# prajwaljpj/GUAVA_renderer

Measured on AMD Instinct MI355X. Metric: rendered frames/sec @512x512, ~100k Gaussians, higher is better.
Workload: dtype f32; 1 GPU; guava-avatar-synth-100k-512-deform+raster; pipeline=EHM LBS -> Gaussian assembly -> rasterize, gaussians=100000, channels=32, global_batch=32, parallelism=frame-sharded x1, batches_in_flight=4, placement=shared, exp=exact-poly, colour_accum=f32 mfma (bit-exact)

## Files before the change

guava_renderer_amd/_lib.py:

```python
import ctypes
import os

HERE = os.path.dirname(os.path.abspath(__file__))
LIB_PATH = os.path.join(HERE, "lib", "libgsr.so")

EXPORTS = ("gsr_version", "gsr_last_error", "gsr_geometry_bytes",
           "gsr_image_bytes", "gsr_binning_bytes", "gsr_mark_visible", "gsr_forward", "gsr_forward_ex",
           "gsr_forward_async_bound", "gsr_forward_async",
           "gsr_backward", "gsr_backward_ex", "gsr_batch_workspace_bytes", "gsr_forward_batch",
           "gsr_backward_batch", "gsr_backward_batch_shared", "gsr_batch_status", "gsr_profile_enable", "gsr_profile_read",
           "gsr_render_counters", "gsr_render_timeline", "gsr_forward_batch_refine", "gsr_render_variant",
           "gsr_refine_prepare", "gsr_batch_status_offset", "gsr_frames_to8b",
           "gsr_refine_backward_scratch_bytes", "gsr_refine_backward_image", "gsr_refine_backward_rows",
           "gsr_stream_create_cu_mask", "gsr_stream_destroy", "gsr_set_render_stream",
           "gsr_lbs_workspace_bytes", "gsr_lbs", "gsr_lbs_sp", "gsr_blend_joints", "gsr_blend_joints_sp",
           "gsr_lbs_tiled_floats", "gsr_lbs_tile_bases",
           "gsr_scratch_geometry", "gsr_scratch_binning", "gsr_scratch_image", "gsr_forward_batch_deformed",
           "gsr_forward_batch_deformed_refine",
           "gsr_splice_head",
           "gsr_pack_rows", "gsr_deform_gaussians", "gsr_ehm_workspace_bytes", "gsr_ehm_forward",
           "gsr_deform_gaussians_backward", "gsr_backward_batch_deformed",
           "gsr_fused_ssim", "gsr_fused_ssim_backward", "gsr_image_loss_partials", "gsr_image_loss",
           "gsr_guava_loss_workspace_bytes", "gsr_guava_loss_partials", "gsr_guava_loss_forward",
           "gsr_guava_loss_backward", "gsr_uv_regularizers_partials", "gsr_uv_regularizers",
           "gsr_mesh_raster_workspace_bytes", "gsr_mesh_raster", "gsr_mesh_visible_texels",
           "gsr_mesh_raster_stats",
           "gsr_lift_vertices", "gsr_lift_uv", "gsr_lift_backward_workspace_bytes",
           "gsr_lift_vertices_backward", "gsr_lift_uv_backward")

NUMERICS_EXACT = 0
NUMERICS_FAST_EXP = 1
NUMERICS_SPLIT_BF16 = 2
FORWARD_ONLY = 0x100
RENDER_VARIANTS = ("strip", "strip_fwd", "split_frame", "split_shared", "split_shared_fwd", "refine", "refine_fwd",
                   "quad", "quad_refine", "half", "half_split", "stats", "timeline", "quad_timeline")


def numerics(fast_exp=False, split_bf16=False):
    return (NUMERICS_FAST_EXP if fast_exp else 0) | (NUMERICS_SPLIT_BF16 if split_bf16 else 0)


ALLOC_FN = ctypes.CFUNCTYPE(ctypes.c_void_p, ctypes.c_void_p, ctypes.c_size_t)

_vp = ctypes.c_void_p
_i = ctypes.c_int
_i64 = ctypes.c_int64
_f = ctypes.c_float
_sz = ctypes.c_size_t
_u32 = ctypes.c_uint32

_lib = None


class RefineEpilogue(ctypes.Structure):
    _fields_ = [("weight", _vp), ("bias", _vp), ("n_out", _i), ("negative_slope", _f),
                ("out_refine", _vp), ("keep_channels", _i)]


class RefineBackwardDesc(ctypes.Structure):
    _fields_ = [("weight", _vp), ("n_out", _i), ("keep_channels", _i), ("negative_slope", _f), ("pad_", _i),
                ("out_refine", _vp), ("dL_dout_refine", _vp), ("dL_dkeep", _vp), ("dL_dprepared", _vp),
                ("scratch", _vp)]


class Scratch(ctypes.Structure):
    _fields_ = [("geometry", _vp), ("geometry_cap", _sz), ("binning", _vp), ("binning_cap", _sz),
                ("image", _vp), ("image_cap", _sz)]


class DeformInputs(ctypes.Structure):
    _fields_ = [("V", _i), ("F", _i), ("N", _i), ("pad_", _i), ("verts", _vp), ("vert_transforms", _vp),
                ("faces", _vp), ("vtx_rotations", _vp), ("vtx_rot_stride", _i64), ("vtx_scales", _vp),
                ("vtx_scale_stride", _i64), ("binding_face", _vp), ("face_bary", _vp), ("local_xyz", _vp),
                ("local_stride", _i64), ("uv_rotations", _vp), ("uv_rot_stride", _i64), ("uv_scales", _vp),
                ("uv_scale_stride", _i64), ("bad_index_flag", _vp)]


class DeformGrads(ctypes.Structure):
    _fields_ = [("vtx_rotations", _vp), ("vtx_scales", _vp), ("local_xyz", _vp), ("uv_rotations", _vp),
                ("uv_scales", _vp)]


class RowSegment(ctypes.Structure):
    _fields_ = [("src", _vp), ("dst", _vp), ("src_stride", _i64), ("dst_stride", _i64), ("width", _i),
                ("pad_", _i)]


class LbsSparse(ctypes.Structure):
    _fields_ = [("jreg_row", _vp), ("jreg_col", _vp), ("jreg_val", _vp), ("skin_k", ctypes.c_int32),
                ("pad_", ctypes.c_int32), ("skin_joint", _vp), ("skin_weight", _vp),
                ("shapedirs_tiled", _vp), ("posedirs_tiled", _vp), ("shapedirs_tiled_k", ctypes.c_int32),
                ("shapedirs_tiled_m", ctypes.c_int32), ("posedirs_tiled_k", ctypes.c_int32),
                ("posedirs_tiled_m", ctypes.c_int32)]


class EhmModel(ctypes.Structure):
    _fields_ = [("V", ctypes.c_int32), ("J", ctypes.c_int32), ("NB", ctypes.c_int32), ("pad_", ctypes.c_int32),
                ("v_template", _vp), ("shapedirs_t", _vp), ("posedirs", _vp), ("J_regressor", _vp),
                ("lbs_weights_t", _vp), ("parents_host", _vp), ("sparse", ctypes.POINTER(LbsSparse))]


class Ehm(ctypes.Structure):
    _fields_ = [("flame", EhmModel), ("body", EhmModel), ("head_index", _vp), ("l_eyelid", _vp),
                ("r_eyelid", _vp), ("N_head", ctypes.c_int32), ("hj0", ctypes.c_int32), ("hj1", ctypes.c_int32),
                ("bj0", ctypes.c_int32), ("bj1", ctypes.c_int32), ("pad_", ctypes.c_int32), ("bad_index_flag", _vp)]


class EhmParam(ctypes.Structure):
    _fields_ = [("p", _vp), ("row_stride", _i64), ("width", ctypes.c_int32), ("pad_", ctypes.c_int32)]


class EhmOutputs(ctypes.Structure):
    _fields_ = [("vertices", _vp), ("joints", _vp), ("joints_transform", _vp), ("ver_transform_mat", _vp),
                ("joint_transform_mat", _vp)]


EHM_SLOTS = ("flame.shape_params", "flame.expression_params", "flame.jaw_params", "flame.eye_pose_params",
             "flame.eyelid_params", "body.shape", "body.exp", "body.global_pose", "body.body_pose",
             "body.left_hand_pose", "body.right_hand_pose", "body.head_scale", "body.joints_offset")


class GsrError(RuntimeError):
    pass


class CapacityError(GsrError):
    """A batched forward needed more Gaussian-tile instances than its workspace holds (that call's
    images were filled with NaN)."""


def load(path=None):
    global _lib
    if _lib is not None:
        return _lib
    path = path or os.environ.get("GSR_LIB") or LIB_PATH
    import torch
    if not os.path.exists(path):
        try:
            from . import build as _build
            _build.build(verbose=False)
        except Exception as e:
            raise GsrError(f"libgsr.so not found at {path} and could not be built: {e}") from e
    L = ctypes.CDLL(path)
    L.gsr_version.restype = ctypes.c_char_p
    built = L.gsr_version().decode().split()[-1]
    if path == LIB_PATH and os.environ.get("GSR_ALLOW_STALE") != "1":
        from . import build as _build
        if os.path.isdir(_build.CSRC) and built != _build.source_hash():
            raise GsrError(f"{path} was built from other sources (hash {built}, tree {_build.source_hash()}): "
                           "rebuild with `python -m guava_renderer_amd.build` (GSR_ALLOW_STALE=1 overrides)")
    L.gsr_last_error.restype = ctypes.c_char_p
    L.gsr_geometry_bytes.argtypes = [_i, _i, _i]
    L.gsr_geometry_bytes.restype = _sz
    L.gsr_image_bytes.argtypes = [_i, _i]
    L.gsr_image_bytes.restype = _sz
    L.gsr_binning_bytes.argtypes = [_i64]
    L.gsr_binning_bytes.restype = _sz
    L.gsr_mark_visible.argtypes = [_i, _vp, _vp, _vp, _vp, _vp]
    L.gsr_mark_visible.restype = _i
    L.gsr_forward.argtypes = [ALLOC_FN, ALLOC_FN, ALLOC_FN, _vp, _i, _i, _i, _vp, _i, _i, _vp, _vp,
                              _vp, _vp, _vp, _f, _vp, _vp, _vp, _vp, _vp, _f, _f, _i, _vp, _vp, _i,
                              _vp, _i, _vp]
    L.gsr_forward.restype = _i
    L.gsr_forward_ex.argtypes = list(L.gsr_forward.argtypes[:-1]) + [_u32, _vp]
    L.gsr_forward_ex.restype = _i
    L.gsr_forward_async_bound.argtypes = [_i, _i, _i]
    L.gsr_forward_async_bound.restype = _i64
    L.gsr_forward_async.argtypes = list(L.gsr_forward.argtypes[:-1]) + [_vp, _u32, _vp]
    L.gsr_forward_async.restype = _i
    L.gsr_backward.argtypes = [_i, _i, _i, _i, _vp, _i, _i, _vp, _vp, _vp, _vp, _vp, _f, _vp, _vp,
                               _vp, _vp, _vp, _f, _f, _vp, _vp, _vp, _vp, _vp, _vp, _vp, _vp, _vp,
                               _vp, _vp, _vp, _vp, _vp, _vp, _vp, _i, _i, _vp]
    L.gsr_backward.restype = _i
    L.gsr_backward_ex.argtypes = list(L.gsr_backward.argtypes[:-1]) + [_u32, _vp]
    L.gsr_backward_ex.restype = _i
    L.gsr_batch_workspace_bytes.argtypes = [_i, _i, _i, _i, _i64]
    L.gsr_batch_workspace_bytes.restype = _sz
    L.gsr_batch_status_offset.argtypes = [_i, _i, _i, _i, _i64]
    L.gsr_batch_status_offset.restype = _sz
    L.gsr_forward_batch.argtypes = [_i, _i, _i, _i, _vp, _i64, _vp, _i64, _vp, _i64, _vp, _i64, _vp,
                                    _i64, _f, _vp, _vp, _vp, _vp, _i64, _vp, _i64, _vp, _vp, _vp, _i,
                                    _u32, _vp]
    L.gsr_forward_batch.restype = _i
    L.gsr_forward_batch_refine.argtypes = list(L.gsr_forward_batch.argtypes[:-2]) + [
        ctypes.POINTER(RefineEpilogue), _u32, _vp]
    L.gsr_forward_batch_refine.restype = _i
    L.gsr_forward_batch_deformed.argtypes = [_i, _i, _i, ctypes.POINTER(DeformInputs), _vp, _i64, _vp, _i64, _f,
                                             _vp, _vp, _vp, _vp, _i64, _vp, _i64, _vp, _vp, _vp, _i, _u32, _vp]
    L.gsr_forward_batch_deformed.restype = _i
    L.gsr_forward_batch_deformed_refine.argtypes = list(L.gsr_forward_batch_deformed.argtypes[:-2]) + [
        ctypes.POINTER(RefineEpilogue), _u32, _vp]
    L.gsr_forward_batch_deformed_refine.restype = _i
    L.gsr_render_variant.argtypes = [_i, _u32, _i]
    L.gsr_render_variant.restype = _i
    L.gsr_refine_prepare.argtypes = [_i, _vp, _vp, _i, _i, _vp, _vp]
    L.gsr_refine_prepare.restype = _i
    L.gsr_refine_backward_scratch_bytes.argtypes = [_i, _i, _i, _i, _i]
    L.gsr_refine_backward_scratch_bytes.restype = _sz
    L.gsr_refine_backward_image.argtypes = [_i, _i, _i, _i, _vp, _i64, ctypes.POINTER(RefineBackwardDesc), _vp]
    L.gsr_refine_backward_image.restype = _i
    L.gsr_refine_backward_rows.argtypes = [_i, _i, _vp, _vp, _i64, _i, _vp, _vp, _i64,
                                           ctypes.POINTER(RefineBackwardDesc), _vp, _vp, _vp, _vp]
    L.gsr_refine_backward_rows.restype = _i
    L.gsr_backward_batch.argtypes = [_i, _i, _i, _i, _vp, _i64, _vp, _i64, _vp, _i64, _vp, _i64, _vp,
                                     _i64, _f, _vp, _vp, _vp, _vp, _i64, _vp, _i64, _vp, _vp, _vp, _vp,
                                     _vp, _vp, _vp, _vp, _vp, _vp, _vp, _i, _u32, _vp]
    L.gsr_backward_batch.restype = _i
    L.gsr_backward_batch_shared.argtypes = list(L.gsr_backward_batch.argtypes[:24]) + [_vp, _vp, _vp, _vp, _vp,
                                                                                       _i, _u32, _vp]
    L.gsr_backward_batch_shared.restype = _i
    L.gsr_batch_status.argtypes = [_vp, _i, _i, ctypes.POINTER(_i64), ctypes.POINTER(_i), _vp]
    L.gsr_batch_status.restype = _i
    L.gsr_profile_enable.argtypes = [ctypes.c_uint32]
    L.gsr_profile_enable.restype = _i
    L.gsr_profile_read.argtypes = [ctypes.POINTER(ctypes.c_double), ctypes.POINTER(_i), _i]
    L.gsr_profile_read.restype = _i
    L.gsr_render_counters.argtypes = [_vp]
    L.gsr_render_counters.restype = _i
    L.gsr_render_timeline.argtypes = [_vp, ctypes.c_uint32]
    L.gsr_render_timeline.restype = _i
    L.gsr_frames_to8b.argtypes = [_i, _i, _i, _i, _vp, _i64, _vp, _vp]
    L.gsr_frames_to8b.restype = _i
    L.gsr_stream_create_cu_mask.argtypes = [_u32, ctypes.POINTER(_u32), ctypes.POINTER(_vp)]
    L.gsr_stream_create_cu_mask.restype = _i
    L.gsr_stream_destroy.argtypes = [_vp]
    L.gsr_stream_destroy.restype = _i
    L.gsr_set_render_stream.argtypes = [_vp, _vp]
    L.gsr_set_render_stream.restype = _i
    L.gsr_lbs_workspace_bytes.argtypes = [_i, _i, _i, _i]
    L.gsr_lbs_workspace_bytes.restype = _sz
    L.gsr_lbs_tiled_floats.argtypes = [_i, _i]
    L.gsr_lbs_tiled_floats.restype = _sz
    L.gsr_lbs_tile_bases.argtypes = [_i, _i, _vp, _vp, _vp]
    L.gsr_lbs_tile_bases.restype = _i
    L.gsr_lbs.argtypes = [_i, _i, _i, _i, _vp, _i64, _vp, _vp, _vp, _i, _vp, _vp, _vp, _vp, _vp, _vp,
                          _vp, _vp, _vp, _vp, _vp, _vp, _vp]
    L.gsr_lbs.restype = _i
    L.gsr_lbs_sp.argtypes = [_i, _i, _i, _i, _vp, _i64, _vp, _vp, _vp, _i, _vp, _vp, _vp, _vp, _vp, _vp,
                             _vp, _vp, _vp, _vp, _vp, _vp, ctypes.POINTER(LbsSparse), _vp]
    L.gsr_lbs_sp.restype = _i
    L.gsr_blend_joints.argtypes = [_i, _i, _i, _i, _vp, _i64, _vp, _vp, _vp, _vp, _vp, _vp, _vp]
    L.gsr_blend_joints.restype = _i
    L.gsr_blend_joints_sp.argtypes = [_i, _i, _i, _i, _vp, _i64, _vp, _vp, _vp, _vp, _vp, _vp,
                                      ctypes.POINTER(LbsSparse), _vp]
    L.gsr_blend_joints_sp.restype = _i
    L.gsr_splice_head.argtypes = [_i, _i, _i, _vp, _vp, _vp, _vp, _vp, _vp, _vp, _i, _i, _i, _vp, _i,
                                  _i, _i, _vp, _vp, _vp]
    L.gsr_splice_head.restype = _i
    L.gsr_pack_rows.argtypes = [_i, _i, ctypes.POINTER(RowSegment), _vp]
    L.gsr_pack_rows.restype = _i
    L.gsr_deform_gaussians.argtypes = [_i, _i, _i, _i, _vp, _vp, _vp, _vp, _i64, _vp, _i64, _vp, _vp,
                                       _vp, _i64, _vp, _i64, _vp, _i64, _vp, _vp, _vp, _vp, _vp]
    L.gsr_deform_gaussians.restype = _i
    L.gsr_deform_gaussians_backward.argtypes = [_i, ctypes.POINTER(DeformInputs), _vp, _vp, _vp,
                                                ctypes.POINTER(DeformGrads), _vp]
    L.gsr_deform_gaussians_backward.restype = _i
    L.gsr_backward_batch_deformed.argtypes = [_i, _i, _i, ctypes.POINTER(DeformInputs), _vp, _vp, _vp, _vp, _i64,
                                              _vp, _i64, _f, _vp, _vp, _vp, _vp, _i64, _vp, _i64, _vp, _vp, _vp,
                                              _vp, ctypes.POINTER(DeformGrads), _i, _u32, _vp]
    L.gsr_backward_batch_deformed.restype = _i
    L.gsr_ehm_workspace_bytes.argtypes = [ctypes.POINTER(Ehm), _i]
    L.gsr_ehm_workspace_bytes.restype = _sz
    L.gsr_ehm_forward.argtypes = [ctypes.POINTER(Ehm), _i, ctypes.POINTER(EhmParam), ctypes.POINTER(EhmOutputs),
                                  _vp, _vp]
    L.gsr_ehm_forward.restype = _i
    L.gsr_fused_ssim.argtypes = [_i, _i, _i, _i, _f, _f, _vp, _vp, _vp, _vp, _vp, _vp, _vp]
    L.gsr_fused_ssim.restype = _i
    L.gsr_fused_ssim_backward.argtypes = [_i, _i, _i, _i, _f, _f, _vp, _vp, _vp, _vp, _vp, _vp, _vp, _vp]
    L.gsr_fused_ssim_backward.restype = _i
    L.gsr_image_loss_partials.argtypes = [_i, _i, _i]
    L.gsr_image_loss_partials.restype = _i
    L.gsr_image_loss.argtypes = [_i, _i, _i, _vp, _vp, _vp, _f, _f, _vp, _vp, _vp, _vp]
    L.gsr_image_loss.restype = _i
    L.gsr_guava_loss_workspace_bytes.argtypes = [_i, _i, _i, _i, _i]
    L.gsr_guava_loss_workspace_bytes.restype = _sz
    L.gsr_guava_loss_partials.argtypes = [_i, _i, _i, _i, _i]
    L.gsr_guava_loss_partials.restype = _i
    L.gsr_guava_loss_forward.argtypes = [_i, _i, _i, _vp, _vp, _vp, _f, _f, _vp, _f, _i, _i, _i, _vp, _vp, _vp,
                                         _vp, _vp, _vp, _vp, _vp]
    L.gsr_guava_loss_forward.restype = _i
    L.gsr_guava_loss_backward.argtypes = [_i, _i, _i, _vp, _f, _f, _vp, _i, _i, _i, _vp, _vp, _vp, _vp, _vp, _vp]
    L.gsr_guava_loss_backward.restype = _i
    L.gsr_uv_regularizers_partials.argtypes = [_i]
    L.gsr_uv_regularizers_partials.restype = _i
    L.gsr_uv_regularizers.argtypes = [_i, _vp, _vp, _f, _f, _f, _f, _vp, _vp, _vp, _vp]
    L.gsr_uv_regularizers.restype = _i
    L.gsr_mesh_raster_workspace_bytes.argtypes = [_i, _i, _i, _i, _i]
    L.gsr_mesh_raster_workspace_bytes.restype = _sz
    L.gsr_mesh_raster.argtypes = [_i, _i, _i, _i, _i, _vp, _vp, _vp, _vp, _vp, _i, _vp, _vp, _vp, _vp, _vp, _vp]
    L.gsr_mesh_raster.restype = _i
    L.gsr_mesh_visible_texels.argtypes = [_i, _i, _i, _vp, _vp, _vp, _vp]
    L.gsr_mesh_visible_texels.restype = _i
    L.gsr_mesh_raster_stats.argtypes = [_vp, ctypes.POINTER(_i64)]
    L.gsr_mesh_raster_stats.restype = _i
    L.gsr_lift_vertices.argtypes = [_i] * 5 + [_vp] * 8
    L.gsr_lift_vertices.restype = _i
    L.gsr_lift_uv.argtypes = [_i] * 7 + [_vp] * 11
    L.gsr_lift_uv.restype = _i
    L.gsr_lift_backward_workspace_bytes.argtypes = [_i, _i, _i, _i]
    L.gsr_lift_backward_workspace_bytes.restype = _sz
    L.gsr_lift_vertices_backward.argtypes = [_i] * 5 + [_vp] * 8
    L.gsr_lift_vertices_backward.restype = _i
    L.gsr_lift_uv_backward.argtypes = [_i] * 7 + [_vp] * 12
    L.gsr_lift_uv_backward.restype = _i
    _lib = L
    return L


def render_variant(B, numerics=0, refine=False):
    return RENDER_VARIANTS[check(load().gsr_render_variant(int(B), int(numerics), int(bool(refine))),
                                 "gsr_render_variant")]


def check(rc, what):
    if rc < 0:
        msg = load().gsr_last_error().decode(errors="replace")
        raise GsrError(f"{what} failed ({-rc}): {msg}")
    return rc
```

guava_renderer_amd/batch.py:

```python
import ctypes
import weakref

import torch

from . import _lib

C = 32
STAGES = ("preprocess", "scan", "depth_sort", "chunk_count", "tile_scan", "ordered_scatter", "render_fwd",
          "render_bwd", "preprocess_bwd")


def _frame_arg(t, B, P, per, name, device, align16=False):
    if not isinstance(t, torch.Tensor):
        raise TypeError(f"{name} must be a tensor")
    if t.device != device:
        raise ValueError(f"{name} must be on {device} (got {t.device})")
    if t.dtype != torch.float32:
        raise TypeError(f"{name} must be float32 (got {t.dtype})")
    if t.dim() == 2:
        if tuple(t.shape) != (P, per):
            raise ValueError(f"{name}: expected [{P},{per}] or [{B},{P},{per}], got {list(t.shape)}")
        t = t.contiguous()
        return t, 0
    if t.dim() != 3 or tuple(t.shape) != (B, P, per):
        raise ValueError(f"{name}: expected [{P},{per}] or [{B},{P},{per}], got {list(t.shape)}")
    if t.stride(0) == 0:
        row = t[0]
        if not row.is_contiguous():
            row = row.contiguous()
        return row, 0
    dense_rows = t.stride(2) == 1 and (t.stride(1) == per or P == 1)
    fs = t.stride(0)
    if not dense_rows or fs < P * per or (align16 and (fs % 4 or t.data_ptr() % 16)):
        t = t.contiguous()
        fs = P * per
    return t, fs


def _frame_mat(t, B, n, name, device):
    if t.device != device or t.dtype != torch.float32:
        raise ValueError(f"{name} must be float32 on {device}")
    if t.numel() != B * n:
        raise ValueError(f"{name}: expected {B}x{n} floats, got shape {list(t.shape)}")
    return t.contiguous()


class BatchRasterizer:

    def __init__(self, B, P, W, H, R_capacity=None, device="cuda", numerics=0):
        self.B, self.P, self.W, self.H = int(B), int(P), int(W), int(H)
        self.device = torch.device(device)
        if self.device.type == "cuda" and self.device.index is None:
            self.device = torch.device("cuda", torch.cuda.current_device())
        self.R_capacity = int(R_capacity if R_capacity is not None else 16 * P * B)
        self.numerics = int(numerics)
        self.L = _lib.load()
        nbytes = self.L.gsr_batch_workspace_bytes(self.B, self.P, self.W, self.H, self.R_capacity)
        soff = self.L.gsr_batch_status_offset(self.B, self.P, self.W, self.H, self.R_capacity)
        self.workspace = torch.empty((nbytes,), dtype=torch.uint8, device=self.device)
        self._sticky = self.workspace[soff:soff + 16].view(torch.int32)
        self._sticky.zero_()
        self._overflow = self.workspace[4:8].view(torch.int32).reshape(())
        self._status_host = torch.zeros(4, dtype=torch.int32, pin_memory=True)
        self._status_ev = None
        self._fwd_count = 0
        self.out_color = torch.empty((self.B, C, self.H, self.W), dtype=torch.float32, device=self.device)
        self.out_invdepth = torch.empty((self.B, self.H, self.W), dtype=torch.float32, device=self.device)
        self.radii = torch.empty((self.B, self.P), dtype=torch.int32, device=self.device)

    def _stream(self):
        return ctypes.c_void_p(torch.cuda.current_stream(self.device).cuda_stream)

    def _inputs(self, means3D, colors, opacities, scales, rotations, viewmatrices, projmatrices,
                tanfov, backgrounds):
        B, P, dev = self.B, self.P, self.device
        none = (None, 0)
        m, sm = none if means3D is None else _frame_arg(means3D, B, P, 3, "means3D", dev)
        c, sc = _frame_arg(colors, B, P, C, "colors", dev, align16=True)
        o, so = _frame_arg(opacities, B, P, 1, "opacities", dev)
        s, ss = none if scales is None else _frame_arg(scales, B, P, 3, "scales", dev)
        r, sr = none if rotations is None else _frame_arg(rotations, B, P, 4, "rotations", dev)
        v = _frame_mat(viewmatrices, B, 16, "viewmatrices", dev)
        pm = _frame_mat(projmatrices, B, 16, "projmatrices", dev)
        tf = _frame_mat(tanfov, B, 2, "tanfov", dev)
        if backgrounds.device != dev or backgrounds.dtype != torch.float32:
            raise ValueError(f"backgrounds must be float32 on {dev}")
        if backgrounds.dim() == 2:
            if tuple(backgrounds.shape) != (B, C):
                raise ValueError(f"backgrounds: expected [{C}] or [{B},{C}], got {list(backgrounds.shape)}")
            bg = backgrounds.contiguous() if backgrounds.stride(0) != 0 else backgrounds[0].contiguous()
            bs = C if backgrounds.stride(0) != 0 else 0
        elif tuple(backgrounds.shape) == (C,):
            bg, bs = backgrounds.contiguous(), 0
        else:
            raise ValueError(f"backgrounds: expected [{C}] or [{B},{C}], got {list(backgrounds.shape)}")
        keep = (m, c, o, s, r, v, pm, tf, bg)
        ptr = lambda t: None if t is None else t.data_ptr()
        args = (B, P, self.W, self.H, ptr(m), sm, c.data_ptr(), sc, o.data_ptr(), so, ptr(s), ss, ptr(r), sr)
        return keep, args, (v.data_ptr(), pm.data_ptr(), tf.data_ptr(), bg.data_ptr(), bs)

    def _after_forward(self):
        self._fwd_count += 1
        self._status_host.copy_(self._sticky, non_blocking=True)
        ev = torch.cuda.Event()
        ev.record(torch.cuda.current_stream(self.device))
        self._status_ev = ev

    def poll(self, wait=False):
        ev = self._status_ev
        if ev is None:
            return
        if wait:
            ev.synchronize()
        elif not ev.query():
            return
        if int(self._status_host[0]):
            rmax = int(self._status_host[1]) & 0xFFFFFFFF
            self.overflow_need = max(getattr(self, "overflow_need", 0), rmax)
            self._sticky.zero_()
            self._status_host.zero_()
            raise _lib.CapacityError(
                f"batch needed {rmax} Gaussian-tile instances, workspace holds {self.R_capacity} "
                f"(that forward's images are NaN); allocate a BatchRasterizer with a larger R_capacity")

    def max_instances_seen(self):
        return max(int(self._status_host[1]) & 0xFFFFFFFF, getattr(self, "overflow_need", 0))

    def overflow_flag(self):
        return self._overflow

    def forward(self, means3D, colors, opacities, scales, rotations, viewmatrices, projmatrices,
                tanfov, backgrounds, scale_modifier=1.0, antialiasing=False, refine=None, numerics=None,
                forward_only=False):
        self.poll()
        nm = self.numerics if numerics is None else int(numerics)
        if forward_only:
            nm |= _lib.FORWARD_ONLY
        self._fwd_only = bool(forward_only)
        keep, head, (v, pm, tf, bg, bs) = self._inputs(means3D, colors, opacities, scales, rotations,
                                                       viewmatrices, projmatrices, tanfov, backgrounds)
        args = head + (float(scale_modifier), v, pm, tf, bg, bs, self.workspace.data_ptr(), self.R_capacity,
                       self.out_color.data_ptr(), self.out_invdepth.data_ptr(), self.radii.data_ptr(),
                       int(bool(antialiasing)))
        if refine is None:
            _lib.check(self.L.gsr_forward_batch(*args, nm, self._stream()), "gsr_forward_batch")
        else:
            pc = refine.prepare(keep[1], self._stream())
            bgrows = keep[8].reshape(-1, C)
            pb = refine.prepare(bgrows, self._stream(), cache=False)
            args = list(args)
            args[6] = pc.data_ptr()
            args[18] = pb.data_ptr()
            ep = refine.epilogue(self.B, self.H, self.W)
            _lib.check(self.L.gsr_forward_batch_refine(*args, ctypes.byref(ep), nm, self._stream()),
                       "gsr_forward_batch_refine")
        del keep
        self._after_forward()
        return self.out_color, self.out_invdepth, self.radii

    def forward_deformed(self, deformer, verts, vert_transforms, viewmatrices, projmatrices, tanfov, backgrounds,
                         scale_modifier=1.0, antialiasing=False, numerics=None, refine=None):
        self.poll()
        nm = self.numerics if numerics is None else int(numerics)
        self._fwd_only = True
        dfm = deformer
        B, P = self.B, self.P
        if dfm.V + dfm.N != P:
            raise ValueError(f"deformer has {dfm.V + dfm.N} Gaussians, the rasterizer {P}")
        if tuple(verts.shape) != (B, dfm.V, 3) or tuple(vert_transforms.shape) != (B, dfm.V, 4, 4):
            raise ValueError("verts / vert_transforms: expected [B,V,3] / [B,V,4,4]")
        for name, t_ in (("verts", verts), ("vert_transforms", vert_transforms), ("deformer.faces", dfm.faces),
                         ("deformer.colors", dfm.colors), ("deformer.bind", dfm.bind)):
            if t_.device != self.device:
                raise ValueError(f"{name} is on {t_.device}, the rasterizer on {self.device}")
        vb = verts.detach().to(torch.float32).contiguous()
        vt = vert_transforms.detach().to(torch.float32).contiguous()
        keep, head, (v, pm, tf, bg, bs) = self._inputs(None, dfm.colors, dfm.opacity, None, None, viewmatrices,
                                                       projmatrices, tanfov, backgrounds)
        di = _lib.DeformInputs(dfm.V, dfm.faces.shape[0], dfm.N, 0, vb.data_ptr(), vt.data_ptr(),
                               dfm.faces.data_ptr(), dfm.v_rot.data_ptr(), 0, dfm.v_scale.data_ptr(), 0,
                               dfm.bind.data_ptr(), dfm.bary.data_ptr(), dfm.u_local.data_ptr(), 0,
                               dfm.u_rot.data_ptr(), 0, dfm.u_scale.data_ptr(), 0, dfm.bad.data_ptr())
        args = (B, self.W, self.H, ctypes.byref(di), head[6], head[7], head[8], head[9], float(scale_modifier),
                v, pm, tf, bg, bs, self.workspace.data_ptr(), self.R_capacity, self.out_color.data_ptr(),
                self.out_invdepth.data_ptr(), self.radii.data_ptr(), int(bool(antialiasing)))
        if refine is None:
            _lib.check(self.L.gsr_forward_batch_deformed(*args, nm, self._stream()), "gsr_forward_batch_deformed")
        else:
            pc = refine.prepare(keep[1], self._stream())
            pb = refine.prepare(keep[8].reshape(-1, C), self._stream(), cache=False)
            args = list(args)
            args[4] = pc.data_ptr()
            args[12] = pb.data_ptr()
            ep = refine.epilogue(B, self.H, self.W)
            _lib.check(self.L.gsr_forward_batch_deformed_refine(*args, ctypes.byref(ep), nm, self._stream()),
                       "gsr_forward_batch_deformed_refine")
        del keep, vb, vt
        self._after_forward()
        return self.out_color, self.out_invdepth, self.radii

    def backward(self, means3D, colors, opacities, scales, rotations, viewmatrices, projmatrices,
                 tanfov, backgrounds, dL_dcolor, dL_dinvdepth=None, scale_modifier=1.0,
                 antialiasing=False, shared=False, numerics=None):
        B, P = self.B, self.P
        if getattr(self, "_fwd_only", False):
            raise _lib.GsrError("backward after forward(forward_only=True): the workspace holds no backward rows")
        nm = self.numerics if numerics is None else int(numerics)
        o = dict(dtype=torch.float32, device=self.device)
        keep, head, (v, pm, tf, bg, bs) = self._inputs(means3D, colors, opacities, scales, rotations,
                                                       viewmatrices, projmatrices, tanfov, backgrounds)
        if tuple(dL_dcolor.shape) != (B, C, self.H, self.W):
            raise ValueError(f"dL_dcolor: expected [{B},{C},{self.H},{self.W}], got {list(dL_dcolor.shape)}")
        dLc = dL_dcolor.to(torch.float32).contiguous()
        dLi = None
        if dL_dinvdepth is not None:
            if dL_dinvdepth.numel() != B * self.H * self.W:
                raise ValueError("dL_dinvdepth: expected [B,H,W]")
            dLi = dL_dinvdepth.to(torch.float32).contiguous()
        if shared:
            strides = head[5::2]
            if any(st_ != 0 for st_ in strides):
                raise ValueError("backward(shared=True) needs attributes shared by every frame "
                                 "([P,k] tensors or frame stride 0); got per-frame inputs")
            g = dict(colors=torch.zeros((P, C), **o), opacity=torch.empty((P, 1), **o),
                     means3D=torch.empty((P, 3), **o), scales=torch.empty((P, 3), **o),
                     rotations=torch.empty((P, 4), **o))
            rc = self.L.gsr_backward_batch_shared(
                *head, float(scale_modifier), v, pm, tf, bg, bs, self.workspace.data_ptr(), self.R_capacity,
                dLc.data_ptr(), dLi.data_ptr() if dLi is not None else None, g["opacity"].data_ptr(),
                g["colors"].data_ptr(), g["means3D"].data_ptr(), g["scales"].data_ptr(),
                g["rotations"].data_ptr(), int(bool(antialiasing)), nm, self._stream())
            _lib.check(rc, "gsr_backward_batch_shared")
            del keep
            return g
        g = dict(mean2D=torch.zeros((B, P, 3), **o), conic=torch.zeros((B, P, 4), **o),
                 opacity=torch.zeros((B, P, 1), **o), colors=torch.zeros((B, P, C), **o),
                 invdepth=torch.zeros((B, P, 1), **o) if dL_dinvdepth is not None else None,
                 means3D=torch.zeros((B, P, 3), **o), cov3D=torch.zeros((B, P, 6), **o),
                 scales=torch.zeros((B, P, 3), **o), rotations=torch.zeros((B, P, 4), **o))
        rc = self.L.gsr_backward_batch(
            *head, float(scale_modifier), v, pm, tf, bg, bs, self.workspace.data_ptr(), self.R_capacity,
            dLc.data_ptr(), dLi.data_ptr() if dLi is not None else None,
            g["mean2D"].data_ptr(), g["conic"].data_ptr(), g["opacity"].data_ptr(),
            g["colors"].data_ptr(), g["invdepth"].data_ptr() if g["invdepth"] is not None else None,
            g["means3D"].data_ptr(), g["cov3D"].data_ptr(), g["scales"].data_ptr(),
            g["rotations"].data_ptr(), int(bool(antialiasing)), nm, self._stream())
        _lib.check(rc, "gsr_backward_batch")
        del keep
        return g

    def _bg_arg(self, backgrounds):
        if backgrounds.device != self.device or backgrounds.dtype != torch.float32:
            raise ValueError(f"backgrounds must be float32 on {self.device}")
        if tuple(backgrounds.shape) == (C,):
            return backgrounds.contiguous().reshape(1, C), 0
        if backgrounds.dim() != 2 or tuple(backgrounds.shape) != (self.B, C):
            raise ValueError(f"backgrounds: expected [{C}] or [{self.B},{C}], got {list(backgrounds.shape)}")
        if backgrounds.stride(0) == 0:
            return backgrounds[0].contiguous().reshape(1, C), 0
        return backgrounds.contiguous(), C

    def refine_backward_image(self, head, dL_drefined, dL_draw=None, out_refine=None):
        B, P, H, W = self.B, self.P, self.H, self.W
        if getattr(self, "_fwd_only", False):
            raise _lib.GsrError("backward after a forward-only forward: the workspace holds no backward rows")
        out = head.out if out_refine is None else out_refine
        if out is None or tuple(out.shape) != (B, head.n_out, H, W):
            raise ValueError(f"out_refine: expected the refine forward's [{B},{head.n_out},{H},{W}] output")
        if tuple(dL_drefined.shape) != (B, head.n_out, H, W):
            raise ValueError(f"dL_drefined: expected [{B},{head.n_out},{H},{W}], got {list(dL_drefined.shape)}")
        if out.device != self.device or dL_drefined.device != self.device:
            raise ValueError(f"out_refine / dL_drefined must be on {self.device}")
        out = out.to(torch.float32).contiguous()
        dout = dL_drefined.to(torch.float32).contiguous()
        dkeep = None
        if dL_draw is not None and head.keep_channels > 0:
            if tuple(dL_draw.shape) != (B, head.keep_channels, H, W) or dL_draw.device != self.device:
                raise ValueError(f"dL_draw: expected [{B},{head.keep_channels},{H},{W}] on {self.device}")
            dkeep = dL_draw.to(torch.float32).contiguous()
        nbytes = max(self.L.gsr_refine_backward_scratch_bytes(B, W, H, P, 1),
                     self.L.gsr_refine_backward_scratch_bytes(B, W, H, B * P, B))
        scratch = torch.empty((nbytes,), dtype=torch.uint8, device=self.device)
        G = torch.empty((B, C, H, W), dtype=torch.float32, device=self.device)
        desc = _lib.RefineBackwardDesc(head.weight.data_ptr(), head.n_out, head.keep_channels, head.slope, 0,
                                       out.data_ptr(), dout.data_ptr(),
                                       dkeep.data_ptr() if dkeep is not None else None, G.data_ptr(),
                                       scratch.data_ptr())
        _lib.check(self.L.gsr_refine_backward_image(B, P, W, H, self.workspace.data_ptr(), self.R_capacity,
                                                    ctypes.byref(desc), self._stream()),
                   "gsr_refine_backward_image")
        del out, dout, dkeep
        return G, scratch

    def refine_backward_rows(self, head, d_prepared, raw_rows, backgrounds, scratch):
        B, P, dev = self.B, self.P, self.device
        raw, rs = _frame_arg(raw_rows, B, P, C, "raw_rows", dev, align16=True)
        if d_prepared.dtype != torch.float32 or d_prepared.device != dev or \
                tuple(d_prepared.shape) not in ((P, C), (B, P, C)):
            raise ValueError(f"d_prepared: expected float32 [{P},{C}] or [{B},{P},{C}] on {dev}")
        frames = 1 if d_prepared.dim() == 2 else B
        if frames == 1 and rs != 0:
            raise ValueError("frame-reduced d_prepared [P,32] needs raw rows shared by every frame")
        dp = d_prepared.contiguous()
        bg, bs = self._bg_arg(backgrounds)
        need = self.L.gsr_refine_backward_scratch_bytes(B, self.W, self.H, dp.numel() // C, frames)
        if scratch.numel() < need:
            raise ValueError("scratch is not the one refine_backward_image returned for this rasterizer")
        o = dict(dtype=torch.float32, device=dev)
        rows = torch.empty_like(dp)
        dW = torch.empty((head.n_out, C), **o)
        db = torch.empty((head.n_out,), **o)
        desc = _lib.RefineBackwardDesc(head.weight.data_ptr(), head.n_out, head.keep_channels, head.slope, 0,
                                       None, None, None, None, scratch.data_ptr())
        _lib.check(self.L.gsr_refine_backward_rows(dp.numel() // C, frames, dp.data_ptr(), raw.data_ptr(), rs, B,
                                                   scratch.data_ptr(), bg.data_ptr(), bs, ctypes.byref(desc),
                                                   rows.data_ptr(), dW.data_ptr(), db.data_ptr(), self._stream()),
                   "gsr_refine_backward_rows")
        del raw, bg, dp
        return rows, dW, db

    def _prepared(self, head, colors, backgrounds):
        raw, _ = _frame_arg(colors, self.B, self.P, C, "colors", self.device, align16=True)
        bg, bs = self._bg_arg(backgrounds)
        pc = head.prepare(raw, self._stream())
        pb = head.prepare(bg, self._stream(), cache=False)
        return pc, (pb if bs else pb[0])

    def backward_refine(self, head, means3D, colors, opacities, scales, rotations, viewmatrices, projmatrices,
                        tanfov, backgrounds, dL_drefined, dL_draw=None, dL_dinvdepth=None, scale_modifier=1.0,
                        antialiasing=False, shared=False, numerics=None, out_refine=None):
        G, scratch = self.refine_backward_image(head, dL_drefined, dL_draw, out_refine)
        pc, pb = self._prepared(head, colors, backgrounds)
        g = self.backward(means3D, pc, opacities, scales, rotations, viewmatrices, projmatrices, tanfov, pb, G,
                          dL_dinvdepth, scale_modifier=scale_modifier, antialiasing=antialiasing, shared=shared,
                          numerics=numerics)
        g["colors"], g["weight"], g["bias"] = self.refine_backward_rows(head, g["colors"], colors, backgrounds,
                                                                        scratch)
        return g

    def backward_deformed(self, deformer, verts, vert_transforms, deformed, colors, opacities, viewmatrices,
                          projmatrices, tanfov, backgrounds, dL_dcolor=None, dL_dinvdepth=None, scale_modifier=1.0,
                          antialiasing=False, numerics=None, refine=None, dL_drefined=None, dL_draw=None):
        if refine is not None:
            if dL_drefined is None or dL_dcolor is not None:
                raise ValueError("backward_deformed(refine=head) takes dL_drefined (and dL_draw), not dL_dcolor")
            G, scratch = self.refine_backward_image(refine, dL_drefined, dL_draw)
            pc, pb = self._prepared(refine, colors, backgrounds)
            g = self.backward_deformed(deformer, verts, vert_transforms, deformed, pc, opacities, viewmatrices,
                                       projmatrices, tanfov, pb, G, dL_dinvdepth, scale_modifier=scale_modifier,
# ... 194 lines not shown
```

guava_renderer_amd/csrc/capi.hip:

```cpp
#include <cstdio>
#include <cstdlib>
#include <cstring>
#include <mutex>
#include <string>
#include <unordered_map>
#include <vector>

#include "../../include/gsr.h"
#include "../../include/gsr_deform.h"

#include "gsr_internal.h"

using namespace gsr;

namespace {

thread_local std::string g_err;
uint64_t* g_render_counters = nullptr;
uint32_t* g_timeline = nullptr;
uint32_t g_timeline_cap = 0;

int fail(gsr_status st, const std::string& msg) {
    g_err = msg;
    return -(int)st;
// ... 16 lines not shown

constexpr int kStages = GSR_NUM_STAGES;
uint32_t g_prof_mask = 0;
struct EvPair { hipEvent_t a, b; int stage; };
std::vector<EvPair> g_ev_pool;
size_t g_ev_used = 0;
double g_prof_ms[kStages] = {0};
int g_prof_cnt[kStages] = {0};

struct StageTimer {
    EvPair* p = nullptr;
    hipStream_t s;
    StageTimer(int stage, hipStream_t st) : s(st) {
        if (!(g_prof_mask & (1u << stage))) return;
        if (g_ev_used == g_ev_pool.size()) {
            EvPair e;
            if (hipEventCreate(&e.a) != hipSuccess || hipEventCreate(&e.b) != hipSuccess) return;
            g_ev_pool.push_back(e);
        }
        p = &g_ev_pool[g_ev_used++];
        p->stage = stage;
        hipEventRecord(p->a, s);
    }
    ~StageTimer() {
        if (p) hipEventRecord(p->b, s);
    }
};

inline bool exact_exp(uint32_t numerics) { return (numerics & GSR_NUMERICS_FAST_EXP) == 0; }
inline bool split_bf16(uint32_t numerics) { return (numerics & GSR_NUMERICS_SPLIT_BF16) != 0; }
constexpr uint32_t kNumericsKnown = GSR_NUMERICS_FAST_EXP | GSR_NUMERICS_SPLIT_BF16;
constexpr uint32_t kForwardBatchKnown = kNumericsKnown | GSR_FORWARD_ONLY;

inline size_t align_up(size_t x) { return (x + 255) & ~(size_t)255; }
inline size_t ctrl_words(const Dims& d) { return (size_t)kCtrlWords + (size_t)kFsWords * d.B; }

std::string grid_error(int width, int height) {
    if ((int64_t)((width + 15) / 16) * ((height + 15) / 16) > kMaxTiles) return "image too large";
    size_t need = 0, limit = 0;
    if (!binning_lds_fits(make_dims(1, 1, width, height), &need, &limit))
        return "image too elongated: the binning kernels need " + std::to_string(need) +
               " bytes of LDS per workgroup for its tile grid, the device has " + std::to_string(limit);
    return std::string();
}

template <typename T>
inline T* take(char* base, size_t& off, size_t count) {
    off = align_up(off);
    T* p = base ? reinterpret_cast<T*>(base + off) : nullptr;
    off += sizeof(T) * count;
    return p;
}

}

namespace gsr {

static void env_tuning(Inputs& in) {
    in.xcd_map = strip_order_tile_major() ? (uint32_t)xcd_queue_map() : 0u;
}

int xcd_queue_map() {
    static const int v = tune_env("GSR_XCD_MAP", 2) == 1 ? 1 : 2;
    return v;
}

int strip_order_tile_major() {
    static const int v = tune_env("GSR_STRIP_ORDER_TILE", 1) != 0 ? 1 : 0;
    return v;
}

int persistent_grid(int per_cu) {
    static int cus = 0;
    if (cus == 0) {
        int dev = 0;
        if (hipGetDevice(&dev) != hipSuccess ||
            hipDeviceGetAttribute(&cus, hipDeviceAttributeMultiprocessorCount, dev) != hipSuccess || cus <= 0)
            cus = 256;
    }
    return cus * per_cu;
}

static std::mutex g_cu_mu;
static std::unordered_map<hipStream_t, int> g_stream_cus;

int persistent_grid_on(hipStream_t s, int per_cu) {
    {
        std::lock_guard<std::mutex> lk(g_cu_mu);
        const auto it = g_stream_cus.find(s);
        if (it != g_stream_cus.end()) return it->second * per_cu;
    }
    return persistent_grid(per_cu);
}

size_t carve_geom(char* base, const Dims& d, GeomArena* g) {
    const size_t n = (size_t)d.B * d.P;
    size_t off = 0;
    GeomArena a;
    a.ctrl = take<uint32_t>(base, off, ctrl_words(d));
    a.fstat = a.ctrl ? a.ctrl + kCtrlWords : nullptr;
    a.depth = take<float>(base, off, n);
    a.invdepth = take<float>(base, off, n);
    a.radii = take<int>(base, off, n);
    a.means2D = take<float2>(base, off, n);
    a.cov3D = take<float>(base, off, 6 * n);
    a.conic = take<float4>(base, off, n);
    a.rect = take<uint2>(base, off, n);
    a.rrec = take<float4>(base, off, 2 * n);
    a.tiles = take<uint32_t>(base, off, n);
    a.blocksums = take<uint32_t>(base, off, (size_t)d.B * d.nblk + 1);
    a.blockkey = take<uint32_t>(base, off, (size_t)d.B * d.nblk * 2);
    a.bslot = take<uint32_t>(base, off, n);
    a.bcount = take<uint32_t>(base, off, (size_t)d.B * (d.NB + 1));
    a.bstart = take<uint32_t>(base, off, (size_t)d.B * (d.NB + 1));
    a.skey = take<uint64_t>(base, off, n);
    a.big = take<uint32_t>(base, off, (size_t)d.B * d.NB);
    a.order = take<uint32_t>(base, off, n);
    a.table = take<uint32_t>(base, off, (size_t)d.B * d.nchunk * d.T);
    a.fsplit = take<uint32_t>(base, off, (size_t)d.P * GSR_C);
    a.gterm = take<float>(base, off, n * kGtWords);
    if (g) *g = a;
    return align_up(off) + 256;
}

size_t carve_image(char* base, const Dims& d, ImageArena* im) {
    const size_t npx = (size_t)d.B * d.W * d.H;
    const size_t nt = (size_t)d.B * d.T;
    size_t off = 0;
    ImageArena a;
    a.final_T = take<float>(base, off, npx);
    a.n_contrib = take<uint32_t>(base, off, npx);
    a.ranges = take<uint2>(base, off, nt);
    a.tile_count = take<uint32_t>(base, off, nt);
    a.work_list = take<uint32_t>(base, off, nt);
    a.lpt_hist = take<uint32_t>(base, off, (size_t)d.B * kLptBuckets);
    a.strip_cnt = take<uint32_t>(base, off, (size_t)kStrips * nt);
    a.strip_list = take<uint32_t>(base, off, (size_t)kStrips * nt);
    a.strip_hist = take<uint32_t>(base, off, (size_t)d.B * 8 * kStripBuckets);
    a.strip_list_bwd = take<uint32_t>(base, off, (size_t)kStrips * nt);
    if (im) *im = a;
    return align_up(off) + 256;
}

size_t carve_bin(char* base, int64_t R, BinArena* b, bool qmask) {
    const size_t n = (size_t)(R > 0 ? R : 1);
    size_t off = 0;
    BinArena a;
    a.point_list = take<uint32_t>(base, off, n);
    a.qmask = qmask ? take<uint32_t>(base, off, n) : nullptr;
    if (b) *b = a;
    return align_up(off) + 256;
}

void launch_deform_preprocess(const Dims& d, const Inputs& in, const GeomArena& g, const Outputs& o,
                              const GsrDeformInputs& dg, hipStream_t s);
void launch_preprocess_bwd_deformed(const Dims& d, const Inputs& in, const GeomArena& g, const Grads& gr,
                                    const GsrDeformInputs& dg, const GsrDeformGrads& dgr, hipStream_t s);
int check_deform_inputs(int B, const GsrDeformInputs* dg, const char* who);

}

namespace {

struct RenderRoute {
    hipStream_t render;
    hipEvent_t ready, done;
};
std::mutex g_route_mu;
std::unordered_map<hipStream_t, RenderRoute> g_routes;

bool render_route(hipStream_t s, RenderRoute* r) {
    std::lock_guard<std::mutex> lk(g_route_mu);
    const auto it = g_routes.find(s);
    if (it == g_routes.end()) return false;
    *r = it->second;
    return true;
}

int run_binning_and_render(const Dims& d, const Inputs& in, const GeomArena& g, const ImageArena& im,
                           const BinArena& bn, const Outputs& o, uint32_t numerics, int debug, hipStream_t s) {
    { StageTimer st_(2, s); launch_depth_sort(d, g, s, in.fuse_totals ? in.totals_cap : -1); }
    STAGE(debug, s, "depth_sort");
    { StageTimer st_(3, s); launch_chunk_count(d, g, im, s); }
    STAGE(debug, s, "chunk_count");
    { StageTimer st_(4, s); launch_tile_scan(d, g, im, s); }
    STAGE(debug, s, "tile_scan");
    {
        StageTimer st_(5, s);
        launch_ordered_scatter(d, g, im, bn, s);
        launch_strip_order(d, g, im, bn, s);
    }
    STAGE(debug, s, "ordered_scatter");
    RenderRoute rt;
    const bool routed = render_route(s, &rt);
    hipStream_t rs = s;
    if (routed) {
        HIP_TRY(hipEventRecord(rt.ready, s));
        HIP_TRY(hipStreamWaitEvent(rt.render, rt.ready, 0));
        rs = rt.render;
    }
    { StageTimer st_(6, rs); launch_render_fwd(d, in, g, im, bn, o, exact_exp(numerics), split_bf16(numerics), rs); }
    if (routed) {
        HIP_TRY(hipEventRecord(rt.done, rs));
        HIP_TRY(hipStreamWaitEvent(s, rt.done, 0));
    }
    STAGE(debug, s, "render_fwd");
    return 0;
}

}

int gsr::api_fail(int status, const char* msg) { return fail((gsr_status)status, msg); }

extern "C" {

#ifndef GSR_SRC_HASH
#define GSR_SRC_HASH "unstamped"
#endif
const char* gsr_version(void) { return "gsr-gfx950 0.2 " GSR_SRC_HASH; }
const char* gsr_last_error(void) { return g_err.c_str(); }

size_t gsr_geometry_bytes(int P, int width, int height) {
    return carve_geom(nullptr, make_dims(1, P, width, height), nullptr);
}
size_t gsr_image_bytes(int width, int height) {
    return carve_image(nullptr, make_dims(1, 1, width, height), nullptr);
}
size_t gsr_binning_bytes(int64_t R) { return carve_bin(nullptr, R, nullptr, true); }

static int64_t async_bound(const Dims& d) {
    const int64_t b = (int64_t)d.P * d.T;
    return b < 0x7FFFFFFFll ? b : 0x7FFFFFFFll;
}

int gsr_mark_visible(int P, const float* means3D, const float* viewmatrix, const float* projmatrix,
                     uint8_t* present, void* stream) {
    if (P < 0) return fail(GSR_ERR_ARG, "P < 0");
    launch_mark_visible(P, means3D, viewmatrix, projmatrix, present, (hipStream_t)stream);
    hipError_t e = hipGetLastError();
    if (e != hipSuccess) return fail(GSR_ERR_HIP, std::string("mark_visible: ") + hipGetErrorString(e));
    return 0;
}

static uint32_t* const kNoStatus = reinterpret_cast<uint32_t*>(uintptr_t(1));

static int forward_single(gsr_alloc_fn geometryBuffer, gsr_alloc_fn binningBuffer, gsr_alloc_fn imageBuffer,
                          void* alloc_ctx, int P, int D, int M, const float* background, int width, int height,
                          const float* means3D, const float* shs, const float* colors_precomp,
                          const float* opacities, const float* scales, float scale_modifier,
                          const float* rotations, const float* cov3D_precomp, const float* viewmatrix,
                          const float* projmatrix, const float* cam_pos, float tan_fovx, float tan_fovy,
                          int prefiltered, float* out_color, float* depth, int antialiasing, int* radii,
                          int debug, uint32_t* status_host, uint32_t numerics, hipStream_t s) {
    (void)D; (void)M; (void)shs; (void)cam_pos;
    if (P < 0 || width <= 0 || height <= 0) return fail(GSR_ERR_ARG, "bad P/width/height");
    if (numerics & ~kNumericsKnown) return fail(GSR_ERR_ARG, "unknown numerics flags");
    if (P >= kMaxGaussians) return fail(GSR_ERR_ARG, "P must be < 2^24");
    if (const std::string ge = grid_error(width, height); !ge.empty()) return fail(GSR_ERR_ARG, ge);
    const Dims d = make_dims(1, P, width, height);
    GeomArena g;
    ImageArena im;
    char* gb = geometryBuffer(alloc_ctx, carve_geom(nullptr, d, nullptr));
    if (!gb) return fail(GSR_ERR_ALLOC, "geometryBuffer allocation failed");
    carve_geom(gb, d, &g);
    char* ib = imageBuffer(alloc_ctx, carve_image(nullptr, d, nullptr));
    if (!ib) return fail(GSR_ERR_ALLOC, "imageBuffer allocation failed");
    carve_image(ib, d, &im);
    if (colors_precomp == nullptr)
        return fail(GSR_ERR_NO_COLORS, "For non-RGB, provide precomputed Gaussian colors!");
    if (((uintptr_t)colors_precomp & 15) != 0) return fail(GSR_ERR_ARG, "colors_precomp must be 16-byte aligned");
    if (cov3D_precomp == nullptr && (scales == nullptr || rotations == nullptr))
        return fail(GSR_ERR_ARG, "scales/rotations or cov3D_precomp required");

    Inputs in{};
    env_tuning(in);
    in.means3D = means3D; in.s_means = 0;
    in.scales = scales; in.s_scales = 0;
    in.rot = rotations; in.s_rot = 0;
    in.opac = opacities; in.s_opac = 0;
    in.cov3D_pre = cov3D_precomp; in.s_cov = 0;
    in.colors = colors_precomp; in.s_colors = 0;
    in.view = viewmatrix; in.proj = projmatrix;
    in.tan_dev = nullptr; in.tanx = tan_fovx; in.tany = tan_fovy;
    in.bg = background; in.s_bg = 0;
    in.scale_mod = scale_modifier;
    in.prefiltered = prefiltered; in.antialiasing = antialiasing;
    Outputs o{out_color, depth, radii, g_render_counters, g_timeline, g_timeline_cap};

    in.zero_ctrl = !in.prefiltered && d.P > 0 && d.B > 0;
    if (!in.zero_ctrl) HIP_TRY(hipMemsetAsync(g.ctrl, 0, ctrl_words(d) * 4, s));
    const bool quad = render_uses_quad(d, split_bf16(numerics), o);
    { StageTimer st_(0, s); launch_preprocess(d, in, g, o, s); }
    STAGE(debug, s, "preprocess");
    if (status_host) {
        const int64_t cap = async_bound(d);
        in.fuse_totals = 1;
        in.totals_cap = cap;
        STAGE(debug, s, "scan");
        char* bb = binningBuffer(alloc_ctx, carve_bin(nullptr, cap, nullptr, quad));
        if (!bb) return fail(GSR_ERR_ALLOC, "binningBuffer allocation failed");
        BinArena bn;
        carve_bin(bb, cap, &bn, quad);
        int rc = run_binning_and_render(d, in, g, im, bn, o, numerics, debug, s);
        if (rc < 0) return rc;
        if (status_host != kNoStatus)
            HIP_TRY(hipMemcpyAsync(status_host, g.ctrl, 4 * sizeof(uint32_t), hipMemcpyDeviceToHost, s));
        return 0;
    }
// ... 60 lines not shown
                      int debug, uint32_t* status_host, uint32_t numerics, void* stream) {
    if (!status_host && prefiltered) return fail(GSR_ERR_ARG, "gsr_forward_async: null status_host with prefiltered");
    if (debug) return fail(GSR_ERR_ARG, "gsr_forward_async: debug mode synchronises; use gsr_forward");
    return forward_single(geometryBuffer, binningBuffer, imageBuffer, alloc_ctx, P, D, M, background, width,
                          height, means3D, shs, colors_precomp, opacities, scales, scale_modifier, rotations,
                          cov3D_precomp, viewmatrix, projmatrix, cam_pos, tan_fovx, tan_fovy, prefiltered,
                          out_color, depth, antialiasing, radii, debug, status_host ? status_host : kNoStatus,
                          numerics, (hipStream_t)stream);
}

char* gsr_scratch_geometry(void* scratch, size_t bytes) {
    const gsr_scratch* sc = static_cast<const gsr_scratch*>(scratch);
    return sc && bytes <= sc->geometry_cap ? sc->geometry : nullptr;
}
char* gsr_scratch_binning(void* scratch, size_t bytes) {
    const gsr_scratch* sc = static_cast<const gsr_scratch*>(scratch);
    return sc && bytes <= sc->binning_cap ? sc->binning : nullptr;
}
char* gsr_scratch_image(void* scratch, size_t bytes) {
    const gsr_scratch* sc = static_cast<const gsr_scratch*>(scratch);
    return sc && bytes <= sc->image_cap ? sc->image : nullptr;
}

int gsr_backward_ex(int P, int D, int M, int R, const float* background, int width, int height,
                    const float* means3D, const float* shs, const float* colors_precomp,
                    const float* opacities, const float* scales, float scale_modifier,
                    const float* rotations, const float* cov3D_precomp, const float* viewmatrix,
                    const float* projmatrix, const float* campos, float tan_fovx, float tan_fovy,
                    const int* radii, char* geom_buffer, char* binning_buffer, char* image_buffer,
                    const float* dL_dpix, const float* dL_invdepths, float* dL_dmean2D,
                    float* dL_dconic, float* dL_dopacity, float* dL_dcolor, float* dL_dinvdepth,
                    float* dL_dmean3D, float* dL_dcov3D, float* dL_dsh, float* dL_dscale,
                    float* dL_drot, int antialiasing, int debug, uint32_t numerics, void* stream) {
    (void)D; (void)M; (void)shs; (void)campos; (void)radii; (void)dL_dsh;
    hipStream_t s = (hipStream_t)stream;
    if (numerics & ~kNumericsKnown) return fail(GSR_ERR_ARG, "unknown numerics flags");
    if (P <= 0) return 0;
    if (colors_precomp == nullptr)
        return fail(GSR_ERR_NO_COLORS, "For non-RGB, provide precomputed Gaussian colors!");
    const Dims d = make_dims(1, P, width, height);
    GeomArena g;
    ImageArena im;
    BinArena bn;
    carve_geom(geom_buffer, d, &g);
    carve_image(image_buffer, d, &im);
    carve_bin(binning_buffer, R, &bn, true);
    Inputs in{};
    env_tuning(in);
    in.means3D = means3D;
    in.scales = scales;
    in.rot = rotations;
    in.opac = opacities;
    in.cov3D_pre = cov3D_precomp;
    in.colors = colors_precomp;
    in.view = viewmatrix; in.proj = projmatrix;
    in.tan_dev = nullptr; in.tanx = tan_fovx; in.tany = tan_fovy;
    in.bg = background;
    in.scale_mod = scale_modifier;
    in.antialiasing = antialiasing;
    Grads gr{};
    gr.dL_dpix = dL_dpix;
    gr.dL_dinvdepth = dL_invdepths;
    gr.dL_dmean2D = dL_dmean2D;
    gr.dL_dconic = dL_dconic;
    gr.dL_dopacity = dL_dopacity;
    gr.dL_dcolors = dL_dcolor;
    gr.dL_dinvdepth_g = dL_invdepths ? dL_dinvdepth : nullptr;
    gr.invd = gr.dL_dinvdepth != nullptr && gr.dL_dinvdepth_g != nullptr;
    gr.dL_dmeans3D = dL_dmean3D;
    gr.dL_dcov3D = dL_dcov3D;
    gr.dL_dscale = (cov3D_precomp == nullptr) ? dL_dscale : nullptr;
    gr.dL_drot = (cov3D_precomp == nullptr) ? dL_drot : nullptr;
    { StageTimer st_(7, s); launch_render_bwd(d, in, g, im, bn, gr, exact_exp(numerics), split_bf16(numerics), s); }
    STAGE(debug, s, "render_bwd");
    { StageTimer st_(8, s); launch_preprocess_bwd(d, in, g, gr, s); }
    STAGE(debug, s, "preprocess_bwd");
    return 0;
}

int gsr_backward(int P, int D, int M, int R, const float* background, int width, int height,
                 const float* means3D, const float* shs, const float* colors_precomp,
                 const float* opacities, const float* scales, float scale_modifier,
                 const float* rotations, const float* cov3D_precomp, const float* viewmatrix,
                 const float* projmatrix, const float* campos, float tan_fovx, float tan_fovy,
                 const int* radii, char* geom_buffer, char* binning_buffer, char* image_buffer,
                 const float* dL_dpix, const float* dL_invdepths, float* dL_dmean2D,
                 float* dL_dconic, float* dL_dopacity, float* dL_dcolor, float* dL_dinvdepth,
                 float* dL_dmean3D, float* dL_dcov3D, float* dL_dsh, float* dL_dscale,
                 float* dL_drot, int antialiasing, int debug, void* stream) {
    return gsr_backward_ex(P, D, M, R, background, width, height, means3D, shs, colors_precomp, opacities,
                           scales, scale_modifier, rotations, cov3D_precomp, viewmatrix, projmatrix, campos,
                           tan_fovx, tan_fovy, radii, geom_buffer, binning_buffer, image_buffer, dL_dpix,
                           dL_invdepths, dL_dmean2D, dL_dconic, dL_dopacity, dL_dcolor, dL_dinvdepth,
                           dL_dmean3D, dL_dcov3D, dL_dsh, dL_dscale, dL_drot, antialiasing, debug,
                           GSR_NUMERICS_EXACT, stream);
}

size_t gsr_batch_status_offset(int B, int P, int width, int height, int64_t R_capacity) {
    const Dims d = make_dims(B, P, width, height);
    return carve_geom(nullptr, d, nullptr) + carve_image(nullptr, d, nullptr) +
           carve_bin(nullptr, R_capacity, nullptr, B == 1);
}

size_t gsr_batch_workspace_bytes(int B, int P, int width, int height, int64_t R_capacity) {
    return gsr_batch_status_offset(B, P, width, height, R_capacity) + 256;
}

static void carve_workspace(char* ws, const Dims& d, int64_t R_cap, GeomArena* g, ImageArena* im,
                            BinArena* bn) {
    const size_t gsz = carve_geom(nullptr, d, nullptr);
    const size_t isz = carve_image(nullptr, d, nullptr);
    const size_t bsz = carve_bin(nullptr, R_cap, nullptr, d.B == 1);
    carve_geom(ws, d, g);
    carve_image(ws + gsz, d, im);
    carve_bin(ws + gsz + isz, R_cap, bn, d.B == 1);
    g->sticky = reinterpret_cast<uint32_t*>(ws + gsz + isz + bsz);
}

int gsr_forward_batch(int B, int P, int width, int height, const float* means3D,
                      int64_t means_stride, const float* colors, int64_t colors_stride,
                      const float* opacities, int64_t opac_stride, const float* scales,
                      int64_t scales_stride, const float* rotations, int64_t rot_stride,
                      float scale_modifier, const float* viewmatrices, const float* projmatrices,
                      const float* tanfov, const float* backgrounds, int64_t bg_stride,
                      char* workspace, int64_t R_capacity, float* out_color, float* out_invdepth,
                      int* radii, int antialiasing, uint32_t numerics, void* stream) {
    return gsr_forward_batch_refine(B, P, width, height, means3D, means_stride, colors, colors_stride,
                                    opacities, opac_stride, scales, scales_stride, rotations, rot_stride,
                                    scale_modifier, viewmatrices, projmatrices, tanfov, backgrounds,
                                    bg_stride, workspace, R_capacity, out_color, out_invdepth, radii,
                                    antialiasing, nullptr, numerics, stream);
}

static std::mutex g_ws_mu;
static std::unordered_map<const void*, bool> g_ws_fwd_only;
static void note_workspace(const void* ws, bool fwd_only) {
    std::lock_guard<std::mutex> lk(g_ws_mu);
    g_ws_fwd_only[ws] = fwd_only;
}
static bool workspace_fwd_only(const void* ws) {
    std::lock_guard<std::mutex> lk(g_ws_mu);
    const auto it = g_ws_fwd_only.find(ws);
    return it != g_ws_fwd_only.end() && it->second;
}

static int forward_batch_impl(int B, int P, int width, int height, const float* means3D,
                              int64_t means_stride, const float* colors, int64_t colors_stride,
                              const float* opacities, int64_t opac_stride, const float* scales,
                              int64_t scales_stride, const float* rotations, int64_t rot_stride,
                              float scale_modifier, const float* viewmatrices, const float* projmatrices,
                              const float* tanfov, const float* backgrounds, int64_t bg_stride,
                              char* workspace, int64_t R_capacity, float* out_color, float* out_invdepth,
                              int* radii, int antialiasing, const gsr_refine_epilogue* refine,
                              uint32_t numerics, const GsrDeformInputs* dg, hipStream_t s) {
    if (numerics & ~kForwardBatchKnown) return fail(GSR_ERR_ARG, "unknown numerics flags");
    if (refine) {
        if (!refine->out_refine || refine->n_out < 1 || refine->keep_channels < 0 ||
            refine->keep_channels + refine->n_out > GSR_C)
            return fail(GSR_ERR_ARG, "refine epilogue: out_refine required, n_out >= 1, keep + n_out <= 32");
    }
    if (B <= 0 || P <= 0 || width <= 0 || height <= 0 || !workspace || !tanfov)
        return fail(GSR_ERR_ARG, "bad batch arguments");
    if (const std::string ge = grid_error(width, height); !ge.empty()) return fail(GSR_ERR_ARG, ge);
    if (B > kMaxFrames) return fail(GSR_ERR_ARG, "too many frames per batch");
    if (P >= kMaxGaussians) return fail(GSR_ERR_ARG, "P must be < 2^24");
    if (!colors) return fail(GSR_ERR_NO_COLORS, "For non-RGB, provide precomputed Gaussian colors!");
    if (((uintptr_t)colors & 15) != 0 || ((colors_stride * 4) & 15) != 0)
        return fail(GSR_ERR_ARG, "colors must be 16-byte aligned per frame");
    const Dims d = make_dims(B, P, width, height);
    GeomArena g;
    ImageArena im;
    BinArena bn;
    carve_workspace(workspace, d, R_capacity, &g, &im, &bn);
    Inputs in{};
    env_tuning(in);
    in.means3D = means3D; in.s_means = means_stride;
    in.scales = scales; in.s_scales = scales_stride;
    in.rot = rotations; in.s_rot = rot_stride;
    in.opac = opacities; in.s_opac = opac_stride;
    in.cov3D_pre = nullptr; in.s_cov = 0;
    in.colors = colors; in.s_colors = colors_stride;
    in.view = viewmatrices; in.proj = projmatrices;
    in.tan_dev = tanfov;
    in.bg = backgrounds; in.s_bg = bg_stride;
    in.scale_mod = scale_modifier;
    in.prefiltered = 0; in.antialiasing = antialiasing;
    in.fwd_only = (numerics & GSR_FORWARD_ONLY) != 0 || dg != nullptr;
    note_workspace(workspace, in.fwd_only != 0);
    Outputs o{out_color, out_invdepth, radii, g_render_counters, g_timeline, g_timeline_cap};
    if (refine) {
        o.rb = refine->bias;
        o.out_refine = refine->out_refine;
        o.n_out = refine->n_out;
        o.keep = refine->keep_channels;
        o.slope = refine->negative_slope;
    }
    if (!render_uses_quad(d, split_bf16(numerics), o)) bn.qmask = nullptr;
    in.zero_ctrl = !in.prefiltered && d.P > 0 && d.B > 0;
    if (!in.zero_ctrl) HIP_TRY(hipMemsetAsync(g.ctrl, 0, ctrl_words(d) * 4, s));
    if (dg) {
        StageTimer st_(0, s);
        launch_deform_preprocess(d, in, g, o, *dg, s);
    } else {
        StageTimer st_(0, s);
        launch_preprocess(d, in, g, o, s);
    }
    if (d.B == 1) {
        in.fuse_totals = 1;
        in.totals_cap = R_capacity;
    } else {
        StageTimer st_(1, s);
        launch_scan_blocksums(d, g, R_capacity, s);
    }
    int rc = run_binning_and_render(d, in, g, im, bn, o, numerics, 0, s);
    if (rc < 0) return rc;
    return 0;
}

int gsr_forward_batch_refine(int B, int P, int width, int height, const float* means3D,
                             int64_t means_stride, const float* colors, int64_t colors_stride,
                             const float* opacities, int64_t opac_stride, const float* scales,
                             int64_t scales_stride, const float* rotations, int64_t rot_stride,
                             float scale_modifier, const float* viewmatrices, const float* projmatrices,
                             const float* tanfov, const float* backgrounds, int64_t bg_stride,
                             char* workspace, int64_t R_capacity, float* out_color, float* out_invdepth,
                             int* radii, int antialiasing, const gsr_refine_epilogue* refine,
                             uint32_t numerics, void* stream) {
    return forward_batch_impl(B, P, width, height, means3D, means_stride, colors, colors_stride, opacities,
                              opac_stride, scales, scales_stride, rotations, rot_stride, scale_modifier,
                              viewmatrices, projmatrices, tanfov, backgrounds, bg_stride, workspace, R_capacity,
                              out_color, out_invdepth, radii, antialiasing, refine, numerics, nullptr,
                              (hipStream_t)stream);
}

int gsr_render_variant(int B, uint32_t numerics, int has_refine) {
    if (B < 1 || (numerics & ~kForwardBatchKnown)) return fail(GSR_ERR_ARG, "gsr_render_variant: B >= 1, known flags");
    return select_render_variant(B, split_bf16(numerics), (numerics & GSR_FORWARD_ONLY) != 0, has_refine != 0, true,
                                 g_render_counters != nullptr, g_timeline != nullptr, B == 1);
}

int gsr_forward_batch_deformed(int B, int width, int height, const GsrDeformInputs* dg, const float* colors,
                               int64_t colors_stride, const float* opacities, int64_t opac_stride,
                               float scale_modifier, const float* viewmatrices, const float* projmatrices,
                               const float* tanfov, const float* backgrounds, int64_t bg_stride,
                               char* workspace, int64_t R_capacity, float* out_color, float* out_invdepth,
                               int* radii, int antialiasing, uint32_t numerics, void* stream) {
    return gsr_forward_batch_deformed_refine(B, width, height, dg, colors, colors_stride, opacities, opac_stride,
                                             scale_modifier, viewmatrices, projmatrices, tanfov, backgrounds,
                                             bg_stride, workspace, R_capacity, out_color, out_invdepth, radii,
                                             antialiasing, nullptr, numerics, stream);
}

int gsr_forward_batch_deformed_refine(int B, int width, int height, const GsrDeformInputs* dg, const float* colors,
                                      int64_t colors_stride, const float* opacities, int64_t opac_stride,
                                      float scale_modifier, const float* viewmatrices, const float* projmatrices,
                                      const float* tanfov, const float* backgrounds, int64_t bg_stride,
                                      char* workspace, int64_t R_capacity, float* out_color, float* out_invdepth,
                                      int* radii, int antialiasing, const gsr_refine_epilogue* refine,
                                      uint32_t numerics, void* stream) {
    if (!dg || dg->V < 0 || dg->N < 0 || dg->F < 0 || dg->V + dg->N == 0 || !dg->verts)
        return fail(GSR_ERR_ARG, "gsr_forward_batch_deformed: bad deform inputs");
    if (dg->V > 0 && (!dg->vert_transforms || !dg->vtx_rotations || !dg->vtx_scales))
        return fail(GSR_ERR_ARG, "gsr_forward_batch_deformed: vertex Gaussians need transforms, rotations, scales");
    if (dg->N > 0 && (!dg->faces || !dg->binding_face || !dg->face_bary || !dg->local_xyz || !dg->uv_rotations ||
                      !dg->uv_scales || dg->F == 0))
        return fail(GSR_ERR_ARG, "gsr_forward_batch_deformed: UV Gaussians need faces and binding data");
    auto bad_stride = [](int64_t st, int64_t full) { return st != 0 && st != full; };
    if (bad_stride(dg->vtx_rot_stride, 4LL * dg->V) || bad_stride(dg->vtx_scale_stride, 3LL * dg->V) ||
        bad_stride(dg->local_stride, 3LL * dg->N) || bad_stride(dg->uv_rot_stride, 4LL * dg->N) ||
        bad_stride(dg->uv_scale_stride, 3LL * dg->N))
        return fail(GSR_ERR_ARG, "gsr_forward_batch_deformed: strides must be 0 or a whole frame");
    return forward_batch_impl(B, dg->V + dg->N, width, height, nullptr, 0, colors, colors_stride, opacities,
                              opac_stride, nullptr, 0, nullptr, 0, scale_modifier, viewmatrices, projmatrices,
                              tanfov, backgrounds, bg_stride, workspace, R_capacity, out_color, out_invdepth, radii,
                              antialiasing, refine, numerics | GSR_FORWARD_ONLY, dg, (hipStream_t)stream);
}

int gsr_refine_prepare(int n, const float* rows, const float* weight, int n_out, int keep_channels,
                       float* prepared, void* stream) {
    if (n < 0 || !weight || n_out < 1 || keep_channels < 0 || keep_channels + n_out > GSR_C)
        return fail(GSR_ERR_ARG, "gsr_refine_prepare: need weight, n_out >= 1, keep + n_out <= 32");
    if (n == 0) return 0;
    if (!rows || !prepared || ((uintptr_t)rows & 15) != 0)
        return fail(GSR_ERR_ARG, "gsr_refine_prepare: rows must be 16-byte aligned, prepared non-null");
    launch_refine_prepare(n, rows, weight, n_out, keep_channels, prepared, (hipStream_t)stream);
    hipError_t e = hipGetLastError();
    if (e != hipSuccess) return fail(GSR_ERR_HIP, std::string("refine_prepare: ") + hipGetErrorString(e));
    return 0;
}

static int backward_batch(int B, int P, int width, int height, const float* means3D, int64_t means_stride,
                          const float* colors, int64_t colors_stride, const float* opacities, int64_t opac_stride,
                          const float* scales, int64_t scales_stride, const float* rotations, int64_t rot_stride,
                          float scale_modifier, const float* viewmatrices, const float* projmatrices,
                          const float* tanfov, const float* backgrounds, int64_t bg_stride, char* workspace,
                          int64_t R_capacity, const Grads& grads, int antialiasing, uint32_t numerics,
                          hipStream_t s, const GsrDeformInputs* dg = nullptr, const GsrDeformGrads* dgr = nullptr) {
    if (B <= 0 || P <= 0 || !workspace || !tanfov) return fail(GSR_ERR_ARG, "bad batch arguments");
    if (numerics & ~kNumericsKnown) return fail(GSR_ERR_ARG, "unknown numerics flags");
    if (P >= kMaxGaussians) return fail(GSR_ERR_ARG, "P must be < 2^24");
    if (workspace_fwd_only(workspace))
        return fail(GSR_ERR_ARG, "backward_batch: the workspace's last forward was GSR_FORWARD_ONLY (no backward rows)");
    const Dims d = make_dims(B, P, width, height);
    GeomArena g;
    ImageArena im;
    BinArena bn;
    carve_workspace(workspace, d, R_capacity, &g, &im, &bn);
    Inputs in{};
    env_tuning(in);
    in.means3D = means3D; in.s_means = means_stride;
    in.scales = scales; in.s_scales = scales_stride;
    in.rot = rotations; in.s_rot = rot_stride;
    in.opac = opacities; in.s_opac = opac_stride;
    in.colors = colors; in.s_colors = colors_stride;
    in.view = viewmatrices; in.proj = projmatrices;
    in.tan_dev = tanfov;
    in.bg = backgrounds; in.s_bg = bg_stride;
    in.scale_mod = scale_modifier;
    in.antialiasing = antialiasing;
    { StageTimer st_(7, s); launch_render_bwd(d, in, g, im, bn, grads, exact_exp(numerics), split_bf16(numerics), s); }
    if (dg) {
        StageTimer st_(8, s);
        launch_preprocess_bwd_deformed(d, in, g, grads, *dg, *dgr, s);
    } else {
        StageTimer st_(8, s);
        launch_preprocess_bwd(d, in, g, grads, s);
    }
    hipError_t e = hipGetLastError();
    if (e != hipSuccess) return fail(GSR_ERR_HIP, std::string("backward_batch: ") + hipGetErrorString(e));
    return 0;
}

int gsr_backward_batch(int B, int P, int width, int height, const float* means3D,
                       int64_t means_stride, const float* colors, int64_t colors_stride,
                       const float* opacities, int64_t opac_stride, const float* scales,
                       int64_t scales_stride, const float* rotations, int64_t rot_stride,
                       float scale_modifier, const float* viewmatrices, const float* projmatrices,
                       const float* tanfov, const float* backgrounds, int64_t bg_stride,
                       char* workspace, int64_t R_capacity, const float* dL_dpix,
                       const float* dL_dinvdepth, float* dL_dmean2D, float* dL_dconic,
                       float* dL_dopacity, float* dL_dcolor, float* dL_dinvdepth_g,
                       float* dL_dmean3D, float* dL_dcov3D, float* dL_dscale, float* dL_drot,
                       int antialiasing, uint32_t numerics, void* stream) {
    if (!dL_dpix || !dL_dmean2D || !dL_dconic || !dL_dopacity || !dL_dcolor || !dL_dmean3D || !dL_dcov3D)
        return fail(GSR_ERR_ARG, "backward_batch: null gradient buffer");
    Grads gr{};
    gr.dL_dpix = dL_dpix;
    gr.dL_dinvdepth = dL_dinvdepth;
    gr.dL_dmean2D = dL_dmean2D;
    gr.dL_dconic = dL_dconic;
    gr.dL_dopacity = dL_dopacity;
    gr.dL_dcolors = dL_dcolor;
    gr.dL_dinvdepth_g = dL_dinvdepth ? dL_dinvdepth_g : nullptr;
    gr.invd = dL_dinvdepth != nullptr && dL_dinvdepth_g != nullptr;
    gr.dL_dmeans3D = dL_dmean3D;
    gr.dL_dcov3D = dL_dcov3D;
    gr.dL_dscale = dL_dscale;
    gr.dL_drot = dL_drot;
    return backward_batch(B, P, width, height, means3D, means_stride, colors, colors_stride, opacities,
                          opac_stride, scales, scales_stride, rotations, rot_stride, scale_modifier,
                          viewmatrices, projmatrices, tanfov, backgrounds, bg_stride, workspace, R_capacity, gr,
                          antialiasing, numerics, (hipStream_t)stream);
}

int gsr_backward_batch_shared(int B, int P, int width, int height, const float* means3D,
                              int64_t means_stride, const float* colors, int64_t colors_stride,
                              const float* opacities, int64_t opac_stride, const float* scales,
                              int64_t scales_stride, const float* rotations, int64_t rot_stride,
                              float scale_modifier, const float* viewmatrices, const float* projmatrices,
                              const float* tanfov, const float* backgrounds, int64_t bg_stride,
                              char* workspace, int64_t R_capacity, const float* dL_dpix,
                              const float* dL_dinvdepth, float* dL_dopacity, float* dL_dcolor,
                              float* dL_dmean3D, float* dL_dscale, float* dL_drot, int antialiasing,
                              uint32_t numerics, void* stream) {
    if (!dL_dpix || !dL_dopacity || !dL_dcolor || !dL_dmean3D || !dL_dscale || !dL_drot)
        return fail(GSR_ERR_ARG, "backward_batch_shared: null gradient buffer");
    if (!scales || !rotations) return fail(GSR_ERR_ARG, "backward_batch_shared: needs scales and rotations");
    Grads gr{};
    gr.dL_dpix = dL_dpix;
    gr.dL_dinvdepth = dL_dinvdepth;
    gr.invd = dL_dinvdepth != nullptr;
    gr.reduce = 1;
    gr.dL_dopacity = dL_dopacity;
    gr.dL_dcolors = dL_dcolor;
    gr.dL_dmeans3D = dL_dmean3D;
    gr.dL_dscale = dL_dscale;
    gr.dL_drot = dL_drot;
    return backward_batch(B, P, width, height, means3D, means_stride, colors, colors_stride, opacities,
                          opac_stride, scales, scales_stride, rotations, rot_stride, scale_modifier,
                          viewmatrices, projmatrices, tanfov, backgrounds, bg_stride, workspace, R_capacity, gr,
                          antialiasing, numerics, (hipStream_t)stream);
}

int gsr_backward_batch_deformed(int B, int width, int height, const GsrDeformInputs* dg, const float* means3D,
                                const float* rotations, const float* scales, const float* colors,
                                int64_t colors_stride, const float* opacities, int64_t opac_stride,
                                float scale_modifier, const float* viewmatrices, const float* projmatrices,
                                const float* tanfov, const float* backgrounds, int64_t bg_stride,
                                char* workspace, int64_t R_capacity, const float* dL_dpix,
                                const float* dL_dinvdepth, float* dL_dopacity, float* dL_dcolor,
                                const GsrDeformGrads* grads, int antialiasing, uint32_t numerics,
                                void* stream) {
    if (const int rc = check_deform_inputs(B, dg, "gsr_backward_batch_deformed")) return rc;
    if (dg->V + dg->N == 0) return fail(GSR_ERR_ARG, "gsr_backward_batch_deformed: no Gaussians");
    if (dg->vtx_rot_stride || dg->vtx_scale_stride || dg->local_stride || dg->uv_rot_stride ||
        dg->uv_scale_stride || colors_stride || opac_stride)
        return fail(GSR_ERR_ARG, "gsr_backward_batch_deformed: canonical attributes, colors and opacities must be "
                                 "shared by every frame (stride 0)");
    if (!means3D || !rotations || !scales || !colors || !opacities)
        return fail(GSR_ERR_ARG, "gsr_backward_batch_deformed: needs the deformed attributes, colors and opacities");
    if (!dL_dpix || !dL_dopacity || !dL_dcolor || !grads)
        return fail(GSR_ERR_ARG, "gsr_backward_batch_deformed: null gradient buffer");
    if ((dg->V > 0 && (!grads->vtx_rotations || !grads->vtx_scales)) ||
        (dg->N > 0 && (!grads->local_xyz || !grads->uv_rotations || !grads->uv_scales)))
        return fail(GSR_ERR_ARG, "gsr_backward_batch_deformed: null canonical gradient buffer");
    const int P = dg->V + dg->N;
    Grads gr{};
    gr.dL_dpix = dL_dpix;
    gr.dL_dinvdepth = dL_dinvdepth;
    gr.invd = dL_dinvdepth != nullptr;
    gr.reduce = 1;
    gr.dL_dopacity = dL_dopacity;
    gr.dL_dcolors = dL_dcolor;
    return backward_batch(B, P, width, height, means3D, 3LL * P, colors, 0, opacities, 0, scales, 3LL * P, rotations,
                          4LL * P, scale_modifier, viewmatrices, projmatrices, tanfov, backgrounds, bg_stride,
                          workspace, R_capacity, gr, antialiasing, numerics, (hipStream_t)stream, dg, grads);
}

// ... 179 lines not shown
```

guava_renderer_amd/csrc/deform.hip:

```cpp
#include <climits>
#include <cstdlib>
#include <string>

#include "../../include/gsr.h"
#include "../../include/gsr_deform.h"
#include "deform_dev.h"
#include "deform_internal.h"
#include "gsr_internal.h"
#include "preprocess_dev.h"

namespace gsr {

#ifndef GSR_DEFORM_NOSTORE
#define GSR_DEFORM_NOSTORE 0
#endif

constexpr int kLbsFrames = 16;
constexpr int kLbsSplit = 4;
constexpr int kLbsSplit1 = 16;

struct Parents {
    int8_t p[GSR_LBS_MAX_JOINTS];
};

// ... 856 lines not shown
            if (j0 + u >= J) break;
#pragma unroll
            for (int e = 0; e < 8; e++)
                T2[e] = __builtin_elementwise_fma(f2{w16[u], w16[u]}, A2[8 * (j0 + u) + e], T2[e]);
        }
    }
    float T[16];
#pragma unroll
    for (int e = 0; e < 8; e++) { T[2 * e] = T2[e].x; T[2 * e + 1] = T2[e].y; }
    const float* p = v_posed + ((int64_t)b * V + v) * 3;
    const float x = p[0], y = p[1], z = p[2];
    float* o = verts + ((int64_t)b * V + v) * 3;
#pragma unroll
    for (int r = 0; r < 3; r++) o[r] = T[4 * r] * x + T[4 * r + 1] * y + T[4 * r + 2] * z + T[4 * r + 3] * 1.0f;
    if (vtrans) {
        float4* tv = reinterpret_cast<float4*>(vtrans + ((int64_t)b * V + v) * 16);
        tv[0] = make_float4(T[0], T[1], T[2], T[3]);
        tv[1] = make_float4(T[4], T[5], T[6], T[7]);
        tv[2] = make_float4(T[8], T[9], T[10], T[11]);
        tv[3] = make_float4(T[12], T[13], T[14], T[15]);
    }
}

__global__ __launch_bounds__(256) void k_splice_head(
    int Vb, int Nh, const int32_t* __restrict__ idx, const float* __restrict__ head,
    const float* __restrict__ r_eyelid, const float* __restrict__ l_eyelid,
    const float* __restrict__ eyelid, const float* __restrict__ head_scale,
    const float* __restrict__ hjoints, int Jh, int hj0, int hj1, const float* __restrict__ bjoints,
    int Jb, int bj0, int bj1, float* __restrict__ body, uint32_t* __restrict__ bad) {
    const int b = blockIdx.y;
    const int i = blockIdx.x * blockDim.x + threadIdx.x;
    if (i >= Nh) return;
    const int d = idx[i];
    if (d < 0 || d >= Vb) {
        if (bad) atomicOr(bad, 2u);
        return;
    }
    const float* hj = hjoints + (int64_t)b * Jh * 3;
    const float* bjt = bjoints + (int64_t)b * Jb * 3;
    for (int c = 0; c < 3; c++) {
        float h = head[((int64_t)b * Nh + i) * 3 + c];
        if (eyelid) {
            h = h + r_eyelid[3 * i + c] * eyelid[2 * b + 1];
            h = h + l_eyelid[3 * i + c] * eyelid[2 * b];
        }
        if (head_scale) h = h * head_scale[3 * b + c];
        float hs = 0.f, bs = 0.f;
        for (int j = hj0; j < hj1; j++) hs += hj[3 * j + c];
        for (int j = bj0; j < bj1; j++) bs += bjt[3 * j + c];
        body[((int64_t)b * Vb + d) * 3 + c] = (h - hs / (float)(hj1 - hj0)) + bs / (float)(bj1 - bj0);
    }
}


constexpr int kDeformFrames = 8;
constexpr int kFrStride = 15;

__global__ __launch_bounds__(256) void k_deform_gaussians(
    int B, int fpw, int V, int F, int N, const float* __restrict__ verts, const float* __restrict__ vtrans,
    const int32_t* __restrict__ faces, const float* __restrict__ vrot, int64_t s_vrot,
    const float* __restrict__ vscale, int64_t s_vscale, const int32_t* __restrict__ bind,
    const float* __restrict__ bary, const float* __restrict__ lxyz, int64_t s_lxyz,
    const float* __restrict__ urot, int64_t s_urot, const float* __restrict__ uscale,
    int64_t s_uscale, float* __restrict__ means, float* __restrict__ rots, float* __restrict__ scales,
    uint32_t* __restrict__ bad) {
    __shared__ float fr_lds[256 * kFrStride];
    __shared__ int range[2];
    const int P = V + N;
    const int i = blockIdx.x * blockDim.x + threadIdx.x;
    const bool uv = i >= V && i < P;
    const int n = i - V;
    int f = -1, j0 = 0, j1 = 0, j2 = 0;
    if (uv) {
        const int bf = bind[n];
        if (bf >= 0 && bf < F) {
            const int a = faces[3 * bf], c = faces[3 * bf + 1], d = faces[3 * bf + 2];
            if (a >= 0 && a < V && c >= 0 && c < V && d >= 0 && d < V) { f = bf; j0 = a; j1 = c; j2 = d; }
        }
        if (f < 0 && bad) atomicOr(bad, 1u);
    }
    float w0 = 0.f, w1 = 0.f, w2 = 0.f;
    if (uv) { w0 = bary[3 * n]; w1 = bary[3 * n + 1]; w2 = bary[3 * n + 2]; }
    if (threadIdx.x == 0) { range[0] = INT_MAX; range[1] = -1; }
    __syncthreads();
    if (f >= 0) { atomicMin(&range[0], f); atomicMax(&range[1], f); }
    __syncthreads();
    const int fmin = range[0], nf = range[1] - range[0] + 1;
    const bool shared_frames = range[1] >= 0 && nf <= 256;
    int t0 = -1, t1 = 0, t2 = 0;
    if (shared_frames && (int)threadIdx.x < nf) {
        const int ff = fmin + threadIdx.x;
        const int a = faces[3 * ff], c = faces[3 * ff + 1], d = faces[3 * ff + 2];
        if (a >= 0 && a < V && c >= 0 && c < V && d >= 0 && d < V) { t0 = a; t1 = c; t2 = d; }
    }
    const int b1 = min(B, (int)(blockIdx.y + 1) * fpw);
    for (int b = blockIdx.y * fpw; b < b1; b++) {
        const float* vb = verts + (int64_t)b * V * 3;
        if (shared_frames) {
            if (b > blockIdx.y * fpw) __syncthreads();
            if (t0 >= 0) face_frame(vb, t0, t1, t2, fr_lds + threadIdx.x * kFrStride);
            __syncthreads();
        }
        if (i >= P) continue;
        const int64_t o = (int64_t)b * P + i;
        if (i < V) {
            const float4* tv = reinterpret_cast<const float4*>(vtrans + ((int64_t)b * V + i) * 16);
            const float4 r0 = tv[0], r1 = tv[1], r2 = tv[2];
            const float m[9] = {r0.x, r0.y, r0.z, r1.x, r1.y, r1.z, r2.x, r2.y, r2.z};
            const float4 qd = rotmat_to_unitquat(m);
            const float* qv = vrot + b * s_vrot + 4 * (int64_t)i;
            const float4 q = quat_product(qd, make_float4(qv[1], qv[2], qv[3], qv[0]));
            const float nn = fmaxf(sqrtf(((q.w * q.w + q.x * q.x) + q.y * q.y) + q.z * q.z), 1e-12f);
            reinterpret_cast<float4*>(rots)[o] = make_float4(q.w / nn, q.x / nn, q.y / nn, q.z / nn);
            for (int c = 0; c < 3; c++) {
                means[3 * o + c] = vb[3 * i + c];
                scales[3 * o + c] = vscale[b * s_vscale + 3 * (int64_t)i + c];
            }
            continue;
        }
        if (f < 0) {
            const float nan = __int_as_float(0x7fc00000);
            for (int c = 0; c < 3; c++) { means[3 * o + c] = nan; scales[3 * o + c] = nan; }
            reinterpret_cast<float4*>(rots)[o] = make_float4(nan, nan, nan, nan);
            continue;
        }
        float fr[14];
        if (shared_frames) {
            const float* src = fr_lds + (f - fmin) * kFrStride;
#pragma unroll
            for (int k = 0; k < 14; k++) fr[k] = src[k];
        } else {
            face_frame(vb, j0, j1, j2, fr);
        }
        const float s = fr[9];
        const float* qu = urot + b * s_urot + 4 * (int64_t)n;
        const float4 q = quat_product(make_float4(fr[10], fr[11], fr[12], fr[13]), make_float4(qu[1], qu[2], qu[3], qu[0]));
        if (!GSR_DEFORM_NOSTORE || q.w == 12345.f) reinterpret_cast<float4*>(rots)[o] = make_float4(q.w, q.x, q.y, q.z);
        const float* l = lxyz + b * s_lxyz + 3 * (int64_t)n;
        const float lx = l[0], ly = l[1], lz = l[2];
        const float cx = (w0 * vb[3 * j0] + w1 * vb[3 * j1]) + w2 * vb[3 * j2];
        const float cy = (w0 * vb[3 * j0 + 1] + w1 * vb[3 * j1 + 1]) + w2 * vb[3 * j2 + 1];
        const float cz = (w0 * vb[3 * j0 + 2] + w1 * vb[3 * j1 + 2]) + w2 * vb[3 * j2 + 2];
        const float mx = dot3(fr[0], fr[1], fr[2], lx, ly, lz) * s + cx;
        const float my = dot3(fr[3], fr[4], fr[5], lx, ly, lz) * s + cy;
        const float mz = dot3(fr[6], fr[7], fr[8], lx, ly, lz) * s + cz;
        const float* us = uscale + b * s_uscale + 3 * (int64_t)n;
        if (!GSR_DEFORM_NOSTORE || mx == 12345.f) {
            means[3 * o] = mx; means[3 * o + 1] = my; means[3 * o + 2] = mz;
            for (int c = 0; c < 3; c++) scales[3 * o + c] = us[c] * s;
        }
    }
}

__global__ __launch_bounds__(256) void k_deform_preprocess(int fpw, GsrDeformInputs dg, Dims d, Inputs in,
                                                           GeomArena g, Outputs o) {
    __shared__ float fr_lds[256 * kFrStride];
    __shared__ int range[2];
    const int V = dg.V, F = dg.F, N = dg.N, P = V + N;
    const int32_t* __restrict__ faces = dg.faces;
    const int i = blockIdx.x * blockDim.x + threadIdx.x;
    const bool uv = i >= V && i < P;
    const int n = i - V;
    int f = -1, j0 = 0, j1 = 0, j2 = 0;
    if (uv) {
        const int bf = dg.binding_face[n];
        if (bf >= 0 && bf < F) {
            const int a = faces[3 * bf], c = faces[3 * bf + 1], e = faces[3 * bf + 2];
            if (a >= 0 && a < V && c >= 0 && c < V && e >= 0 && e < V) { f = bf; j0 = a; j1 = c; j2 = e; }
        }
        if (f < 0 && dg.bad_index_flag) atomicOr(dg.bad_index_flag, 1u);
    }
    float w0 = 0.f, w1 = 0.f, w2 = 0.f;
    if (uv) { w0 = dg.face_bary[3 * n]; w1 = dg.face_bary[3 * n + 1]; w2 = dg.face_bary[3 * n + 2]; }
    if (threadIdx.x == 0) { range[0] = INT_MAX; range[1] = -1; }
    __syncthreads();
    if (f >= 0) { atomicMin(&range[0], f); atomicMax(&range[1], f); }
    __syncthreads();
    const int fmin = range[0], nf = range[1] - range[0] + 1;
    const bool shared_frames = range[1] >= 0 && nf <= 256;
    int t0 = -1, t1 = 0, t2 = 0;
    if (shared_frames && (int)threadIdx.x < nf) {
        const int ff = fmin + threadIdx.x;
        const int a = faces[3 * ff], c = faces[3 * ff + 1], e = faces[3 * ff + 2];
        if (a >= 0 && a < V && c >= 0 && c < V && e >= 0 && e < V) { t0 = a; t1 = c; t2 = e; }
    }
    const int b1 = min(d.B, (int)(blockIdx.y + 1) * fpw);
    for (int b = blockIdx.y * fpw; b < b1; b++) {
        const float* vb = dg.verts + (int64_t)b * V * 3;
        if (shared_frames) {
            if (b > (int)blockIdx.y * fpw) __syncthreads();
            if (t0 >= 0) face_frame(vb, t0, t1, t2, fr_lds + threadIdx.x * kFrStride);
            __syncthreads();
        }
        for (int k = i; k <= d.NB; k += d.nblk * kScanBlock) g.bcount[(int64_t)b * (d.NB + 1) + k] = 0u;
        const int64_t gid = (int64_t)b * P + i;
        uint32_t tiles = 0;
        if (i < P) {
            float mo[3], so[3], qq[4];
            if (i < V) {
                const float4* tv = reinterpret_cast<const float4*>(dg.vert_transforms + ((int64_t)b * V + i) * 16);
                const float4 r0 = tv[0], r1 = tv[1], r2 = tv[2];
                const float m[9] = {r0.x, r0.y, r0.z, r1.x, r1.y, r1.z, r2.x, r2.y, r2.z};
                const float4 qd = rotmat_to_unitquat(m);
                const float* qv = dg.vtx_rotations + b * dg.vtx_rot_stride + 4 * (int64_t)i;
                const float4 q = quat_product(qd, make_float4(qv[1], qv[2], qv[3], qv[0]));
                const float nn = fmaxf(sqrtf(((q.w * q.w + q.x * q.x) + q.y * q.y) + q.z * q.z), 1e-12f);
                qq[0] = q.w / nn; qq[1] = q.x / nn; qq[2] = q.y / nn; qq[3] = q.z / nn;
                for (int c = 0; c < 3; c++) {
                    mo[c] = vb[3 * i + c];
                    so[c] = dg.vtx_scales[b * dg.vtx_scale_stride + 3 * (int64_t)i + c];
                }
            } else if (f < 0) {
                const float nan = __int_as_float(0x7fc00000);
                for (int c = 0; c < 3; c++) { mo[c] = nan; so[c] = nan; }
                for (int c = 0; c < 4; c++) qq[c] = nan;
            } else {
                float fr[14];
                if (shared_frames) {
                    const float* src = fr_lds + (f - fmin) * kFrStride;
#pragma unroll
                    for (int k = 0; k < 14; k++) fr[k] = src[k];
                } else {
                    face_frame(vb, j0, j1, j2, fr);
                }
                const float s = fr[9];
                const float* qu = dg.uv_rotations + b * dg.uv_rot_stride + 4 * (int64_t)n;
                const float4 q = quat_product(make_float4(fr[10], fr[11], fr[12], fr[13]),
                                              make_float4(qu[1], qu[2], qu[3], qu[0]));
                qq[0] = q.w; qq[1] = q.x; qq[2] = q.y; qq[3] = q.z;
                const float* l = dg.local_xyz + b * dg.local_stride + 3 * (int64_t)n;
                const float lx = l[0], ly = l[1], lz = l[2];
                const float cx = (w0 * vb[3 * j0] + w1 * vb[3 * j1]) + w2 * vb[3 * j2];
                const float cy = (w0 * vb[3 * j0 + 1] + w1 * vb[3 * j1 + 1]) + w2 * vb[3 * j2 + 1];
                const float cz = (w0 * vb[3 * j0 + 2] + w1 * vb[3 * j1 + 2]) + w2 * vb[3 * j2 + 2];
                mo[0] = dot3(fr[0], fr[1], fr[2], lx, ly, lz) * s + cx;
                mo[1] = dot3(fr[3], fr[4], fr[5], lx, ly, lz) * s + cy;
                mo[2] = dot3(fr[6], fr[7], fr[8], lx, ly, lz) * s + cz;
                const float* us = dg.uv_scales + b * dg.uv_scale_stride + 3 * (int64_t)n;
                for (int c = 0; c < 3; c++) so[c] = us[c] * s;
            }
            tiles = preprocess_one(d, in, g, o, b, gid, mo, nullptr, so, qq, in.opac[in.s_opac * b + i]);
        }
        preprocess_block_sums(d, g, b, blockIdx.x, tiles, gid);
    }
    zero_ctrl_words(d, in, g);
}

void launch_deform_preprocess(const Dims& d, const Inputs& in, const GeomArena& g, const Outputs& o,
                              const GsrDeformInputs& dg, hipStream_t s) {
    if (d.P == 0 || d.B == 0) return;
    static const int fpw = [] {
        const int v = tune_env("GSR_FUSED_FRAMES", 4);
        return v >= 1 && v <= 64 ? v : 1;
    }();
    hipLaunchKernelGGL(k_deform_preprocess, dim3(d.nblk, (d.B + fpw - 1) / fpw), dim3(256), 0, s, fpw, dg, d, in,
                       g, o);
}

__global__ __launch_bounds__(256) void k_deform_gaussians_bwd(int B, int fpw, GsrDeformInputs dg,
                                                              const float* __restrict__ g_means,
                                                              const float* __restrict__ g_rots,
                                                              const float* __restrict__ g_scales, GsrDeformGrads o) {
    const int V = dg.V, N = dg.N, P = V + N;
    const int i = blockIdx.x * blockDim.x + threadIdx.x;
    if (i >= P) return;
    const int b0 = blockIdx.y * fpw, b1 = min(B, b0 + fpw);
    if (i < V) {
        float ar[4] = {0.f, 0.f, 0.f, 0.f}, as[3] = {0.f, 0.f, 0.f};
        for (int b = b0; b < b1; b++) {
            const int64_t gid = (int64_t)b * P + i;
            if (o.vtx_rotations) {
                const float* qv = dg.vtx_rotations + b * dg.vtx_rot_stride + 4 * (int64_t)i;
                const float q[4] = {qv[0], qv[1], qv[2], qv[3]};
                const float g[4] = {g_rots[4 * gid], g_rots[4 * gid + 1], g_rots[4 * gid + 2], g_rots[4 * gid + 3]};
                float dq[4];
                deform_bwd_vertex_rot(dg.vert_transforms + ((int64_t)b * V + i) * 16, q, g, dq);
                if (dg.vtx_rot_stride) {
#pragma unroll
                    for (int k = 0; k < 4; k++) o.vtx_rotations[b * dg.vtx_rot_stride + 4 * (int64_t)i + k] = dq[k];
                } else {
#pragma unroll
                    for (int k = 0; k < 4; k++) ar[k] += dq[k];
                }
            }
            if (o.vtx_scales) {
#pragma unroll
                for (int k = 0; k < 3; k++) {
                    const float gs = g_scales[3 * gid + k];
                    if (dg.vtx_scale_stride) o.vtx_scales[b * dg.vtx_scale_stride + 3 * (int64_t)i + k] = gs;
                    else as[k] += gs;
                }
            }
        }
        if (o.vtx_rotations && !dg.vtx_rot_stride)
#pragma unroll
            for (int k = 0; k < 4; k++) o.vtx_rotations[4 * (int64_t)i + k] = ar[k];
        if (o.vtx_scales && !dg.vtx_scale_stride)
#pragma unroll
            for (int k = 0; k < 3; k++) o.vtx_scales[3 * (int64_t)i + k] = as[k];
        return;
    }
    const int n = i - V;
    const DeformBinding bd = resolve_binding(dg.binding_face, dg.faces, n, V, dg.F);
    if (bd.f < 0 && dg.bad_index_flag && blockIdx.y == 0) atomicOr(dg.bad_index_flag, 1u);
    float al[3] = {0.f, 0.f, 0.f}, ar[4] = {0.f, 0.f, 0.f, 0.f}, as[3] = {0.f, 0.f, 0.f};
    for (int b = b0; b < b1; b++) {
        const int64_t gid = (int64_t)b * P + i;
        float dl[3] = {0.f, 0.f, 0.f}, dr[4] = {0.f, 0.f, 0.f, 0.f}, ds[3] = {0.f, 0.f, 0.f};
        if (bd.f >= 0) {
            float fr[14];
            face_frame_bwd(dg.verts + (int64_t)b * V * 3, bd.j0, bd.j1, bd.j2, fr);
            float gm[3] = {0.f, 0.f, 0.f}, gq[4] = {0.f, 0.f, 0.f, 0.f}, gs[3] = {0.f, 0.f, 0.f};
            if (o.local_xyz)
#pragma unroll
                for (int k = 0; k < 3; k++) gm[k] = g_means[3 * gid + k];
            if (o.uv_rotations)
#pragma unroll
                for (int k = 0; k < 4; k++) gq[k] = g_rots[4 * gid + k];
            if (o.uv_scales)
#pragma unroll
                for (int k = 0; k < 3; k++) gs[k] = g_scales[3 * gid + k];
            deform_bwd_uv(fr, gm, gq, gs, dl, dr, ds);
        }
        if (o.local_xyz) {
#pragma unroll
            for (int k = 0; k < 3; k++) {
                if (dg.local_stride) o.local_xyz[b * dg.local_stride + 3 * (int64_t)n + k] = dl[k];
                else al[k] += dl[k];
            }
        }
        if (o.uv_rotations) {
#pragma unroll
            for (int k = 0; k < 4; k++) {
                if (dg.uv_rot_stride) o.uv_rotations[b * dg.uv_rot_stride + 4 * (int64_t)n + k] = dr[k];
                else ar[k] += dr[k];
            }
        }
        if (o.uv_scales) {
#pragma unroll
            for (int k = 0; k < 3; k++) {
                if (dg.uv_scale_stride) o.uv_scales[b * dg.uv_scale_stride + 3 * (int64_t)n + k] = ds[k];
                else as[k] += ds[k];
            }
        }
    }
    if (o.local_xyz && !dg.local_stride)
#pragma unroll
        for (int k = 0; k < 3; k++) o.local_xyz[3 * (int64_t)n + k] = al[k];
    if (o.uv_rotations && !dg.uv_rot_stride)
#pragma unroll
        for (int k = 0; k < 4; k++) o.uv_rotations[4 * (int64_t)n + k] = ar[k];
    if (o.uv_scales && !dg.uv_scale_stride)
#pragma unroll
        for (int k = 0; k < 3; k++) o.uv_scales[3 * (int64_t)n + k] = as[k];
}

struct PackTable {
    GsrRowSegment seg[GSR_PACK_MAX_SEGMENTS];
};

__global__ __launch_bounds__(256) void k_pack_rows(PackTable t) {
    const GsrRowSegment sg = t.seg[blockIdx.x];
    const int b = blockIdx.y;
    for (int c = threadIdx.x; c < sg.width; c += 256)
        sg.dst[b * sg.dst_stride + c] = sg.src ? sg.src[b * sg.src_stride + c] : 0.f;
}

namespace {

size_t align256(size_t x) { return (x + 255) & ~(size_t)255; }

struct LbsArena {
    float *rot, *feat, *vs, *vp, *joints, *A;
    float *beta_tiles, *feat_tiles;
};

size_t coef_tile_floats(int B, int K) { return (size_t)((B + 31) / 32) * (size_t)((K + 7) / 8) * 256; }

size_t carve_lbs(char* base, int B, int V, int J, int NB, LbsArena* a) {
    size_t off = 0;
    auto take = [&](size_t bytes) {
        char* p = base ? base + off : nullptr;
        off += align256(bytes);
        return reinterpret_cast<float*>(p);
    };
    const size_t f = sizeof(float);
    LbsArena t;
    t.rot = take(f * (size_t)B * J * 9);
    t.feat = take(f * (size_t)B * (J > 1 ? J - 1 : 1) * 9);
    t.vs = take(f * (size_t)B * V * 3);
    t.vp = take(f * (size_t)B * V * 3);
    t.joints = take(f * (size_t)B * J * 3);
    t.A = take(f * (size_t)B * J * 16);
    t.beta_tiles = take(f * coef_tile_floats(B, NB > 0 ? NB : 0));
    t.feat_tiles = take(f * coef_tile_floats(B, 9 * (J - 1)));
    if (a) *a = t;
    return off;
}

int hip_check(const char* what) {
    hipError_t e = hipGetLastError();
    if (e != hipSuccess) return api_fail(GSR_ERR_HIP, (std::string(what) + ": " + hipGetErrorString(e)).c_str());
    return 0;
}

}

int check_deform_inputs(int B, const GsrDeformInputs* dg, const char* who) {
    auto bad = [&](const char* msg) { return api_fail(GSR_ERR_ARG, (std::string(who) + ": " + msg).c_str()); };
// ... 388 lines not shown
                         const float* eyelid, const float* head_scale, const float* head_joints, int hj0, int hj1,
                         const float* body_joints, int Jb, int bj0, int bj1, float* body_v_shaped,
                         uint32_t* bad_index_flag, void* stream) {
    if (!sp_h || sp_h->skin_k <= 0) return 1;
    if (hj0 < 0 || hj1 <= hj0 || hj1 > Jh || bj0 < 0 || bj1 <= bj0 || bj1 > Jb)
        return api_fail(GSR_ERR_ARG, "gsr_ehm_forward: bad reference joint ranges");
    if (eyelid && (!r_eyelid || !l_eyelid)) return api_fail(GSR_ERR_ARG, "gsr_ehm_forward: eyelid bases missing");
    LbsArena a;
    carve_lbs(const_cast<char*>(ws_h), B, Vh, Jh, 0, &a);
    const dim3 g((Vh + 255) / 256, B);
    hipStream_t s = (hipStream_t)stream;
#define GSR_SKS(KM)                                                                                              \
    hipLaunchKernelGGL(k_skin_splice<KM>, g, dim3(256), 0, s, Vh, Jh, sp_h->skin_k, sp_h->skin_joint,            \
                       sp_h->skin_weight, a.A, a.vp, Vb, head_index, r_eyelid, l_eyelid, eyelid, head_scale,     \
                       head_joints, hj0, hj1, body_joints, Jb, bj0, bj1, body_v_shaped, bad_index_flag)
    if (sp_h->skin_k <= 4) GSR_SKS(4);
    else if (sp_h->skin_k <= 8) GSR_SKS(8);
    else GSR_SKS(16);
#undef GSR_SKS
    return hip_check("skin_splice");
}

extern "C" {

int gsr_blend_joints(int B, int V, int J, int NB, const float* v_template, int64_t v_template_stride,
                     const float* betas, const float* shapedirs_t, const float* J_regressor,
                     const float* joints_offset, float* v_shaped, float* joints, void* stream) {
    return gsr_blend_joints_sp(B, V, J, NB, v_template, v_template_stride, betas, shapedirs_t, J_regressor,
                               joints_offset, v_shaped, joints, nullptr, stream);
}

int gsr_blend_joints_sp(int B, int V, int J, int NB, const float* v_template, int64_t v_template_stride,
                        const float* betas, const float* shapedirs_t, const float* J_regressor,
                        const float* joints_offset, float* v_shaped, float* joints, const GsrLbsSparse* sp,
                        void* stream) {
    return gsr::blend_joints_run(B, V, J, NB, v_template, v_template_stride, betas, shapedirs_t, J_regressor,
                                 joints_offset, v_shaped, joints, sp, stream, false);
}

}

int gsr::blend_joints_run(int B, int V, int J, int NB, const float* v_template, int64_t v_template_stride,
                          const float* betas, const float* shapedirs_t, const float* J_regressor,
                          const float* joints_offset, float* v_shaped, float* joints, const GsrLbsSparse* sp,
                          void* stream, bool blend_done) {
    if (B <= 0 || V <= 0 || J < 1) return api_fail(GSR_ERR_ARG, "gsr_blend_joints: bad sizes");
    if (int rc = check_sparse(sp, 1, betas ? NB : 0, V, "gsr_blend_joints")) return rc;
    if (!v_template || !J_regressor || !v_shaped || !joints)
        return api_fail(GSR_ERR_ARG, "gsr_blend_joints: null required pointer");
    if (v_template_stride != 0 && v_template_stride != (int64_t)V * 3)
        return api_fail(GSR_ERR_ARG, "gsr_blend_joints: v_template stride must be 0 or V*3");
    if (betas && (NB <= 0 || !shapedirs_t))
        return api_fail(GSR_ERR_ARG, "gsr_blend_joints: betas need NB > 0 and shapedirs");
    if (!betas) NB = 0;
    if (lbs_blend_lds(NB, 0, kLbsFrames, kLbsSplit) > 160 * 1024) return api_fail(GSR_ERR_ARG, "gsr_blend_joints: NB too large for LDS");
    hipStream_t s = (hipStream_t)stream;
    const int M = V * 3;
    if (!blend_done) {
        launch_blend(B, M, NB, 0, v_template, v_template_stride, betas, shapedirs_t, nullptr, nullptr, v_shaped, nullptr,
                     s, sp);
        if (int rc = hip_check("blend_shapes")) return rc;
    }
    launch_joints(B, V, J, J_regressor, sp, v_shaped, joints_offset, joints, s);
    return hip_check("vertices2joints");
}

extern "C" {

size_t gsr_lbs_tiled_floats(int K, int M) {
    if (K <= 0 || M <= 0) return 0;
    return (size_t)((M + 31) / 32) * (size_t)((K + 7) / 8) * 256;
}

int gsr_lbs_tile_bases(int K, int M, const float* base, float* tiled, void* stream) {
    if (K <= 0 || M <= 0 || !base || !tiled) return api_fail(GSR_ERR_ARG, "gsr_lbs_tile_bases: bad arguments");
    if (((uintptr_t)tiled & 15) != 0) return api_fail(GSR_ERR_ARG, "gsr_lbs_tile_bases: tiled must be 16-byte aligned");
    const int64_t n4 = (int64_t)gsr_lbs_tiled_floats(K, M) / 4;
    hipLaunchKernelGGL(k_lbs_tile_base, dim3((unsigned)((n4 + 255) / 256)), dim3(256), 0, (hipStream_t)stream, K, M,
                       n4, base, reinterpret_cast<float4*>(tiled));
    return hip_check("lbs_tile_base");
}

int gsr_splice_head(int B, int V_body, int N_head, const int32_t* head_index, const float* head_verts,
                    const float* r_eyelid, const float* l_eyelid, const float* eyelid_params,
                    const float* head_scale, const float* head_joints, int J_head, int hj0, int hj1,
                    const float* body_joints, int J_body, int bj0, int bj1, float* body_v_shaped,
                    uint32_t* bad_index_flag, void* stream) {
    if (B <= 0 || V_body <= 0 || N_head < 0) return api_fail(GSR_ERR_ARG, "gsr_splice_head: bad sizes");
    if (N_head == 0) return 0;
    if (!head_index || !head_verts || !head_joints || !body_joints || !body_v_shaped)
        return api_fail(GSR_ERR_ARG, "gsr_splice_head: null required pointer");
    if (eyelid_params && (!r_eyelid || !l_eyelid))
        return api_fail(GSR_ERR_ARG, "gsr_splice_head: eyelid_params need both eyelid bases");
    if (hj0 < 0 || hj1 <= hj0 || hj1 > J_head || bj0 < 0 || bj1 <= bj0 || bj1 > J_body)
        return api_fail(GSR_ERR_ARG, "gsr_splice_head: bad reference joint ranges");
    hipLaunchKernelGGL(k_splice_head, dim3((N_head + 255) / 256, B), dim3(256), 0, (hipStream_t)stream,
                       V_body, N_head, head_index, head_verts, r_eyelid, l_eyelid, eyelid_params,
                       head_scale, head_joints, J_head, hj0, hj1, body_joints, J_body, bj0, bj1,
                       body_v_shaped, bad_index_flag);
    return hip_check("splice_head");
}

int gsr_pack_rows(int B, int nseg, const GsrRowSegment* segs, void* stream) {
    if (B <= 0 || nseg < 0 || nseg > GSR_PACK_MAX_SEGMENTS) return api_fail(GSR_ERR_ARG, "gsr_pack_rows: bad sizes");
    if (nseg == 0) return 0;
    if (!segs) return api_fail(GSR_ERR_ARG, "gsr_pack_rows: null segment table");
    PackTable t;
    for (int i = 0; i < nseg; i++) {
        t.seg[i] = segs[i];
        if (!segs[i].dst || segs[i].width < 0 || segs[i].width > 4096 || segs[i].dst_stride < segs[i].width ||
            segs[i].src_stride < 0)
            return api_fail(GSR_ERR_ARG, "gsr_pack_rows: bad segment");
    }
    hipLaunchKernelGGL(k_pack_rows, dim3(nseg, B), dim3(256), 0, (hipStream_t)stream, t);
    return hip_check("pack_rows");
}

int gsr_deform_gaussians(int B, int V, int F, int N, const float* verts,
                         const float* vert_transforms, const int32_t* faces,
                         const float* vtx_rotations, int64_t vtx_rot_stride,
                         const float* vtx_scales, int64_t vtx_scale_stride,
                         const int32_t* binding_face, const float* face_bary,
                         const float* local_xyz, int64_t local_stride,
                         const float* uv_rotations, int64_t uv_rot_stride,
                         const float* uv_scales, int64_t uv_scale_stride, float* means3D,
                         float* rotations, float* scales, uint32_t* bad_index_flag, void* stream) {
    if (B <= 0 || V < 0 || N < 0 || F < 0) return api_fail(GSR_ERR_ARG, "gsr_deform_gaussians: bad sizes");
    if (V + N == 0) return 0;
    if (!verts || !means3D || !rotations || !scales)
        return api_fail(GSR_ERR_ARG, "gsr_deform_gaussians: null required pointer");
    if (V > 0 && (!vert_transforms || !vtx_rotations || !vtx_scales))
        return api_fail(GSR_ERR_ARG, "gsr_deform_gaussians: vertex Gaussians need transforms, rotations, scales");
    if (N > 0 && (!faces || !binding_face || !face_bary || !local_xyz || !uv_rotations || !uv_scales || F == 0))
        return api_fail(GSR_ERR_ARG, "gsr_deform_gaussians: UV Gaussians need faces and binding data");
    auto bad_stride = [](int64_t st, int64_t full) { return st != 0 && st != full; };
    if (bad_stride(vtx_rot_stride, 4LL * V) || bad_stride(vtx_scale_stride, 3LL * V) ||
        bad_stride(local_stride, 3LL * N) || bad_stride(uv_rot_stride, 4LL * N) ||
        bad_stride(uv_scale_stride, 3LL * N))
        return api_fail(GSR_ERR_ARG, "gsr_deform_gaussians: strides must be 0 or a whole frame");
    hipStream_t s = (hipStream_t)stream;
    static const int fpw = [] {
        const int v = tune_env("GSR_DEFORM_FRAMES", kDeformFrames);
        return v >= 1 && v <= 64 ? v : 1;
    }();
    const int P = V + N;
    hipLaunchKernelGGL(k_deform_gaussians, dim3((P + 255) / 256, (B + fpw - 1) / fpw), dim3(256), 0, s, B, fpw,
                       V, F, N, verts, vert_transforms, faces, vtx_rotations, vtx_rot_stride, vtx_scales,
                       vtx_scale_stride, binding_face, face_bary, local_xyz, local_stride, uv_rotations,
                       uv_rot_stride, uv_scales, uv_scale_stride, means3D, rotations, scales,
                       bad_index_flag);
    return hip_check("deform_gaussians");
}

int gsr_deform_gaussians_backward(int B, const GsrDeformInputs* dg, const float* dL_dmeans3D,
                                  const float* dL_drotations, const float* dL_dscales,
                                  const GsrDeformGrads* grads, void* stream) {
    const char* who = "gsr_deform_gaussians_backward";
    if (const int rc = check_deform_inputs(B, dg, who)) return rc;
    if (!grads) return api_fail(GSR_ERR_ARG, "gsr_deform_gaussians_backward: null gradient struct");
    const int P = dg->V + dg->N;
    if (P == 0) return 0;
    GsrDeformGrads o = *grads;
    if (dg->V == 0) o.vtx_rotations = o.vtx_scales = nullptr;
    if (dg->N == 0) o.local_xyz = o.uv_rotations = o.uv_scales = nullptr;
    if (!o.vtx_rotations && !o.vtx_scales && !o.local_xyz && !o.uv_rotations && !o.uv_scales) return 0;
    if (((o.vtx_rotations || o.uv_rotations) && !dL_drotations) || ((o.vtx_scales || o.uv_scales) && !dL_dscales) ||
        (o.local_xyz && !dL_dmeans3D))
        return api_fail(GSR_ERR_ARG, "gsr_deform_gaussians_backward: a wanted gradient needs its upstream gradient");
    const bool any_shared = (o.vtx_rotations && !dg->vtx_rot_stride) || (o.vtx_scales && !dg->vtx_scale_stride) ||
                            (o.local_xyz && !dg->local_stride) || (o.uv_rotations && !dg->uv_rot_stride) ||
                            (o.uv_scales && !dg->uv_scale_stride);
    const int fpw = any_shared || B < kDeformFrames ? B : kDeformFrames;
    hipLaunchKernelGGL(k_deform_gaussians_bwd, dim3((P + 255) / 256, (B + fpw - 1) / fpw), dim3(256), 0,
                       (hipStream_t)stream, B, fpw, *dg, dL_dmeans3D, dL_drotations, dL_dscales, o);
    return hip_check("deform_gaussians_backward");
}

}
```

guava_renderer_amd/csrc/preprocess.hip:

```cpp
#include "preprocess_dev.h"

namespace gsr {

__global__ __launch_bounds__(kScanBlock) void k_preprocess(Dims d, Inputs in, GeomArena g, Outputs o) {
    const int b = blockIdx.y;
    const int i = blockIdx.x * kScanBlock + threadIdx.x;
    const int64_t gid = (int64_t)b * d.P + i;
    for (int k = i; k <= d.NB; k += d.nblk * kScanBlock) g.bcount[(int64_t)b * (d.NB + 1) + k] = 0u;
    uint32_t tiles = 0;
    if (i < d.P) {
        const float* pm = in.means3D + in.s_means * b + 3 * (int64_t)i;
        const float p[3] = {pm[0], pm[1], pm[2]};
        const float* cp = in.cov3D_pre ? in.cov3D_pre + in.s_cov * b + 6 * (int64_t)i : nullptr;
        float sc[3] = {0.f, 0.f, 0.f}, q[4] = {0.f, 0.f, 0.f, 0.f};
        if (!cp) {
            const float* sp = in.scales + in.s_scales * b + 3 * (int64_t)i;
            const float* rp = in.rot + in.s_rot * b + 4 * (int64_t)i;
            sc[0] = sp[0]; sc[1] = sp[1]; sc[2] = sp[2];
            q[0] = rp[0]; q[1] = rp[1]; q[2] = rp[2]; q[3] = rp[3];
        }
        tiles = preprocess_one(d, in, g, o, b, gid, p, cp, sc, q, in.opac[in.s_opac * b + i]);
    }
    zero_ctrl_words(d, in, g);
    preprocess_block_sums(d, g, b, blockIdx.x, tiles, gid);
}

void launch_preprocess(const Dims& d, const Inputs& in, const GeomArena& g, const Outputs& o,
                       hipStream_t s) {
    if (d.P == 0 || d.B == 0) return;
    dim3 grid(d.nblk, d.B);
    hipLaunchKernelGGL(k_preprocess, grid, dim3(kScanBlock), 0, s, d, in, g, o);
}

__global__ void k_mark_visible(int P, const float* __restrict__ means3D, const float* view,
                               const float* proj, uint8_t* present) {
    const int i = blockIdx.x * blockDim.x + threadIdx.x;
    if (i >= P) return;
    const float p[3] = {means3D[3 * i], means3D[3 * i + 1], means3D[3 * i + 2]};
    float ph[4];
    xform4x4(p, proj, ph);
    float pv[3];
    xform4x3(p, view, pv);
    present[i] = (pv[2] <= 0.2f) ? 0 : 1;
}

void launch_mark_visible(int P, const float* means3D, const float* view, const float* proj,
                         uint8_t* present, hipStream_t s) {
    if (P <= 0) return;
    hipLaunchKernelGGL(k_mark_visible, dim3((P + 255) / 256), dim3(256), 0, s, P, means3D, view, proj,
                       present);
}

}
```

guava_renderer_amd/csrc/preprocess_dev.h:

```cpp
#pragma once
#include "gsr_internal.h"

namespace gsr {

__device__ __forceinline__ void cov3d_fwd(const float s[3], float mod, const float q[4], float* cov) {
    mat3 S = mk3(1, 0, 0, 0, 1, 0, 0, 0, 1);
    S.m[0][0] = mod * s[0];
    S.m[1][1] = mod * s[1];
    S.m[2][2] = mod * s[2];
    const float r = q[0], x = q[1], y = q[2], z = q[3];
    mat3 R = mk3(1.f - 2.f * (y * y + z * z), 2.f * (x * y - r * z), 2.f * (x * z + r * y),
                 2.f * (x * y + r * z), 1.f - 2.f * (x * x + z * z), 2.f * (y * z - r * x),
                 2.f * (x * z - r * y), 2.f * (y * z + r * x), 1.f - 2.f * (x * x + y * y));
    mat3 M = mul3(S, R);
    mat3 Sig = mul3(tr3(M), M);
    cov[0] = Sig.m[0][0]; cov[1] = Sig.m[0][1]; cov[2] = Sig.m[0][2];
    cov[3] = Sig.m[1][1]; cov[4] = Sig.m[1][2]; cov[5] = Sig.m[2][2];
}

__device__ __forceinline__ uint32_t preprocess_one(const Dims& d, const Inputs& in, const GeomArena& g,
                                                   const Outputs& o, int b, int64_t gid, const float p[3],
                                                   const float* cp, const float sc[3], const float q[4],
                                                   float op) {
    uint32_t tiles = 0;
    const float* view = in.view + 16 * b;
    const float* proj = in.proj + 16 * b;
    const float tanx = in.tan_dev ? in.tan_dev[2 * b] : in.tanx;
    const float tany = in.tan_dev ? in.tan_dev[2 * b + 1] : in.tany;
    const float focal_y = (float)d.H / (2.0f * tany);
    const float focal_x = (float)d.W / (2.0f * tanx);
    int radius = 0;
    uint2 rect = make_uint2(0, 0);
    float ph[4];
    xform4x4(p, proj, ph);
    const float pw = 1.0f / (ph[3] + 0.0000001f);
    float pv[3];
    xform4x3(p, view, pv);
    if (pv[2] <= 0.2f) {
        if (in.prefiltered) atomicOr(&g.ctrl[kCtrlError], 1u);
    } else {
        const float pproj[2] = {ph[0] * pw, ph[1] * pw};
        float c3[6];
        if (cp) {
#pragma unroll
            for (int k = 0; k < 6; k++) c3[k] = cp[k];
        } else {
            cov3d_fwd(sc, in.scale_mod, q, c3);
            if (!in.fwd_only)
#pragma unroll
                for (int k = 0; k < 6; k++) g.cov3D[6 * gid + k] = c3[k];
        }
        float t[3];
        xform4x3(p, view, t);
        const float limx = 1.3f * tanx;
        const float limy = 1.3f * tany;
        const float txtz = t[0] / t[2];
        const float tytz = t[1] / t[2];
        t[0] = fminf(limx, fmaxf(-limx, txtz)) * t[2];
        t[1] = fminf(limy, fmaxf(-limy, tytz)) * t[2];
        const mat3 J = mk3(focal_x / t[2], 0.0f, -(focal_x * t[0]) / (t[2] * t[2]),
                           0.0f, focal_y / t[2], -(focal_y * t[1]) / (t[2] * t[2]), 0, 0, 0);
        const mat3 W = mk3(view[0], view[4], view[8], view[1], view[5], view[9], view[2], view[6],
                           view[10]);
        const mat3 T = mul3(W, J);
        const mat3 V = mk3(c3[0], c3[1], c3[2], c3[1], c3[3], c3[4], c3[2], c3[4], c3[5]);
        const mat3 cv = mul3(mul3(tr3(T), tr3(V)), T);
        float cx = cv.m[0][0], cy = cv.m[0][1], cz = cv.m[1][1];
        const float h_var = 0.3f;
        const float det_cov = cx * cz - cy * cy;
        cx += h_var;
        cz += h_var;
        const float det_cov_plus_h_cov = cx * cz - cy * cy;
        float h_conv = 1.0f;
        if (in.antialiasing) h_conv = sqrtf(fmaxf(0.000025f, det_cov / det_cov_plus_h_cov));
        const float det = det_cov_plus_h_cov;
        if (det != 0.0f) {
            const float det_inv = 1.f / det;
            const float conic0 = cz * det_inv, conic1 = -cy * det_inv, conic2 = cx * det_inv;
            const float mid = 0.5f * (cx + cz);
            const float lambda1 = mid + sqrtf(fmaxf(0.1f, mid * mid - det));
            const float lambda2 = mid - sqrtf(fmaxf(0.1f, mid * mid - det));
            const float my_radius = ceilf(3.f * sqrtf(fmaxf(lambda1, lambda2)));
            const float pix0 = ndc2pix(pproj[0], d.W), pix1 = ndc2pix(pproj[1], d.H);
            uint32_t rmin[2], rmax[2];
            const int ir = f2i(my_radius);
            get_rect(pix0, pix1, ir, d.gx, d.gy, rmin, rmax);
            const uint32_t nt = (rmax[0] - rmin[0]) * (rmax[1] - rmin[1]);
            if (nt != 0) {
                g.depth[gid] = pv[2];
                if (!in.fwd_only) {
                    g.invdepth[gid] = 1.0f / pv[2];
                    g.means2D[gid] = make_float2(pix0, pix1);
                    g.conic[gid] = make_float4(conic0, conic1, conic2, op * h_conv);
                }
                radius = ir;
                tiles = nt;
                rect = make_uint2(rmin[0] | (rmin[1] << 16), rmax[0] | (rmax[1] << 16));
                float4* rr = g.rrec + 2 * gid;
                rr[0] = make_float4(pix0, pix1, op * h_conv, 1.0f / pv[2]);
                rr[1] = make_float4(-0.5f * conic0, -conic1, -0.5f * conic2, 0.f);
            }
        }
    }
    if (!in.fwd_only) g.radii[gid] = radius;
    g.tiles[gid] = tiles;
    g.rect[gid] = rect;
    if (o.radii) o.radii[gid] = radius;
    return tiles;
}

__device__ __forceinline__ void preprocess_block_sums(const Dims& d, const GeomArena& g, int b, int blk_x,
                                                      uint32_t tiles, int64_t gid) {
    __shared__ uint32_t red[3][kScanBlock / 64];
    uint32_t v = tiles;
    const uint32_t key = tiles ? __float_as_uint(g.depth[gid]) : 0u;
    uint32_t kmax = key, nkmax = tiles ? ~key : 0u;
#pragma unroll
    for (int off = 32; off > 0; off >>= 1) {
        v += __shfl_xor(v, off);
        kmax = max(kmax, (uint32_t)__shfl_xor(kmax, off));
        nkmax = max(nkmax, (uint32_t)__shfl_xor(nkmax, off));
    }
    if ((threadIdx.x & 63) == 0) {
        red[0][threadIdx.x >> 6] = v;
        red[1][threadIdx.x >> 6] = kmax;
        red[2][threadIdx.x >> 6] = nkmax;
    }
    __syncthreads();
    if (threadIdx.x == 0) {
        uint32_t s = 0, km = 0, nkm = 0;
#pragma unroll
        for (int w = 0; w < kScanBlock / 64; w++) {
            s += red[0][w];
            km = max(km, red[1][w]);
            nkm = max(nkm, red[2][w]);
        }
        const int64_t blk = (int64_t)b * d.nblk + blk_x;
        g.blocksums[blk] = s;
        g.blockkey[2 * blk] = km;
        g.blockkey[2 * blk + 1] = nkm;
    }
    __syncthreads();
}


__device__ __forceinline__ void zero_ctrl_words(const Dims& d, const Inputs& in, const GeomArena& g) {
    const int64_t t = ((int64_t)blockIdx.y * gridDim.x + blockIdx.x) * blockDim.x + threadIdx.x;
    if (in.zero_ctrl) {
        const int64_t n = (int64_t)kCtrlWords + (int64_t)kFsWords * d.B;
        const int64_t T = (int64_t)gridDim.x * gridDim.y * blockDim.x;
        for (int64_t k = t; k < n; k += T)
            if (k != kCtrlFwdOnly) g.ctrl[k] = 0u;
        if (t == 0) g.ctrl[kCtrlFwdOnly] = in.fwd_only ? 1u : 0u;
    } else if (in.fwd_only && t == 0) {
        g.ctrl[kCtrlFwdOnly] = 1u;
    }
}
}
```

guava_renderer_amd/deform.py:

```python
import ctypes
import os

import numpy as np
import torch

from . import _lib

_T_CACHE = {}


def _dev_check(*ts):
    for t in ts:
        if t is not None and not t.is_cuda:
            raise RuntimeError("guava_renderer_amd.deform runs on the GPU only (got a CPU tensor)")


def _f32(t):
    return t.detach().to(torch.float32).contiguous()


def _cached_t(t, fn):
    key = (t.data_ptr(), tuple(t.shape), t._version, fn.__name__)
    hit = _T_CACHE.get(key)
    if hit is None:
# ... 2 lines not shown
        hit = fn(t)
        _T_CACHE[key] = hit
    return hit


def _shapedirs_t(sd):
    return _f32(sd).permute(2, 0, 1).reshape(sd.shape[2], -1).contiguous()


def _weights_t(w):
    return _f32(w).t().contiguous()


def _ptr(t):
    return ctypes.c_void_p(t.data_ptr()) if t is not None else None


def _stream(dev):
    return ctypes.c_void_p(torch.cuda.current_stream(dev).cuda_stream)


def _parents_host(parents):
    p = parents.detach().cpu().numpy() if torch.is_tensor(parents) else np.asarray(parents)
    return np.ascontiguousarray(p.astype(np.int32))


def _run_lbs(betas, pose, v_template, shapedirs, posedirs, J_regressor, parents, lbs_weights,
             joints_offset, pose2rot, want_all):
    _dev_check(pose, v_template, posedirs, J_regressor, lbs_weights, betas, shapedirs, joints_offset)
    dev = v_template.device
    B = pose.shape[0] if betas is None else max(betas.shape[0], pose.shape[0])
    Jn = J_regressor.shape[0]
    V = J_regressor.shape[1]
    if v_template.shape[-2:] != (V, 3):
        raise RuntimeError(f"v_template must be [.., {V}, 3], got {tuple(v_template.shape)}")
    if lbs_weights.shape != (V, Jn):
        raise RuntimeError(f"lbs_weights must be [{V}, {Jn}], got {tuple(lbs_weights.shape)}")
    vt = _f32(v_template)
    if vt.dim() == 3 and vt.shape[0] == 1 and B > 1:
        vt = vt[0]
    vt_stride = 0 if vt.dim() == 2 else V * 3
    if vt.dim() == 3 and vt.shape[0] != B:
        raise RuntimeError("v_template batch does not match the pose batch")
    pose = _f32(pose)
    if pose2rot:
        if pose.numel() != B * Jn * 3:
            raise RuntimeError(f"pose must hold B*J*3 = {B * Jn * 3} axis-angle values")
    elif pose.numel() != B * Jn * 9:
        raise RuntimeError(f"pose must hold B*J*9 = {B * Jn * 9} rotation-matrix values")
    NB = 0
    sd = None
    bt = None
    if betas is not None:
        NB = betas.shape[1]
        if shapedirs.shape != (V, 3, NB):
            raise RuntimeError(f"shapedirs must be [{V}, 3, {NB}], got {tuple(shapedirs.shape)}")
        sd = _cached_t(shapedirs, _shapedirs_t)
        bt = _f32(betas).expand(B, NB).contiguous()
    if Jn > 1 and posedirs.shape != (9 * (Jn - 1), 3 * V):
        raise RuntimeError(f"posedirs must be [{9 * (Jn - 1)}, {3 * V}], got {tuple(posedirs.shape)}")
    pd = _f32(posedirs)
    jreg = _f32(J_regressor)
    wt = _cached_t(lbs_weights, _weights_t)
    jo = _f32(joints_offset).expand(B, Jn, 3).contiguous() if joints_offset is not None else None
    par = _parents_host(parents)
    o = dict(dtype=torch.float32, device=dev)
    verts = torch.empty((B, V, 3), **o)
    jt = torch.empty((B, Jn, 3), **o)
    jr = torch.empty((B, Jn, 3), **o) if want_all else None
    T = torch.empty((B, V, 4, 4), **o) if want_all else None
    A = torch.empty((B, Jn, 4, 4), **o) if want_all else None
    L = _lib.load()
    ws = torch.empty((L.gsr_lbs_workspace_bytes(B, V, Jn, NB),), dtype=torch.uint8, device=dev)
    rc = L.gsr_lbs(B, V, Jn, NB, _ptr(vt), vt_stride, _ptr(bt), _ptr(sd), _ptr(pose),
                   1 if pose2rot else 0, _ptr(pd), _ptr(jreg),
                   par.ctypes.data_as(ctypes.c_void_p), _ptr(wt), _ptr(jo), _ptr(verts), _ptr(jt),
                   _ptr(jr), _ptr(T), _ptr(A), None, _ptr(ws), _stream(dev))
    _lib.check(rc, "gsr_lbs")
    return verts, jt, jr, T, A


def lbs(betas, pose, v_template, shapedirs, posedirs, J_regressor, parents, lbs_weights,
        joints_offset=None, pose2rot=True, dtype=torch.float32):
    verts, jt, _, _, _ = _run_lbs(betas, pose, v_template, shapedirs, posedirs, J_regressor,
                                  parents, lbs_weights, joints_offset, pose2rot, False)
    return verts, jt


def lbs_wobeta(pose, v_shaped, posedirs, J_regressor, parents, lbs_weights, joints_offset=None,
               pose2rot=True, dtype=torch.float32):
    return _run_lbs(None, pose, v_shaped, None, posedirs, J_regressor, parents, lbs_weights,
                    joints_offset, pose2rot, True)


def _seg(segs, dst, col, t, B, width=None):
    if t is None:
        return
    t = _f32(t)
    rows = t.reshape(t.shape[0], -1) if t.dim() > 1 else t.reshape(1, -1)
    if rows.shape[0] not in (1, B):
        raise RuntimeError(f"parameter batch {rows.shape[0]} does not match the frame batch {B}")
    w = rows.shape[1] if width is None else width
    if w > rows.shape[1] or col + w > dst.shape[1]:
        raise RuntimeError(f"parameter of width {rows.shape[1]} does not fit columns [{col}, {col + w}) "
                           f"of a {dst.shape[1]}-wide coefficient row")
    _dev_check(rows)
    segs.append((rows, dst, col, w, 0 if rows.shape[0] == 1 else rows.stride(0)))


def _fill_zeros(segs, dsts, B):
    table = []
    for rows, dst, col, w, sstr in segs:
        if w > 0:
            table.append(_lib.RowSegment(rows.data_ptr(), dst.data_ptr() + 4 * col, sstr, dst.stride(0), w, 0))
    for dst in dsts:
        covered = sorted((col, col + w) for _, d, col, w, _ in segs if d is dst and w > 0)
        c = 0
        for a, e in covered + [(dst.shape[1], dst.shape[1])]:
            if a < c:
                raise RuntimeError("overlapping coefficient segments")
            if a > c:
                table.append(_lib.RowSegment(None, dst.data_ptr() + 4 * c, 0, dst.stride(0), a - c, 0))
            c = max(c, e)
    if len(table) > 16:
        raise RuntimeError("too many coefficient segments for one gsr_pack_rows launch")
    return table


class GaussianDeformer:

    def __init__(self, vertex_gaussian_assets, uv_gaussian_assets, faces, sh_degree=0,
                 apply_rgb_sigmoid=True):
        va, ua = vertex_gaussian_assets, uv_gaussian_assets

        def sq(t):
            t = t.detach()
            return _f32(t[0] if t.dim() == 3 and t.shape[0] == 1 else t)

        _dev_check(faces, va["rotations"], ua["rotations"])
        self.faces = faces.detach().to(torch.int32).contiguous()
        self.v_rot, self.v_scale = sq(va["rotations"]), sq(va["scales"])
        self.u_rot, self.u_scale = sq(ua["rotations"]), sq(ua["scales"])
        self.u_local = sq(ua["local_pos"])
        self.bind = ua["binding_face"].detach().reshape(-1).to(torch.int32).contiguous()
        self.bary = _f32(ua["face_bary"].detach().reshape(-1, 3))
        self.V, self.N = self.v_rot.shape[0], self.u_rot.shape[0]
        col = torch.cat([sq(va["colors"]), sq(ua["colors"])], 0)
        if apply_rgb_sigmoid:
            col[:, :3] = torch.sigmoid(col[:, :3])
        self.colors = col.contiguous()
        self.opacity = torch.cat([sq(va["opacities"]), sq(ua["opacities"])], 0).contiguous()
        self.sh_degree = sh_degree
        self.bad = torch.zeros(1, dtype=torch.int32, device=self.faces.device)

    def forward(self, verts, vert_transforms):
        _dev_check(verts, vert_transforms)
        B, V = verts.shape[:2]
        if V != self.V:
            raise RuntimeError(f"expected {self.V} vertices, got {V}")
        P = self.V + self.N
        dev = verts.device
        buf = torch.empty((B * P * 10,), dtype=torch.float32, device=dev)
        rot = buf[:B * P * 4].view(B, P, 4)
        xyz = buf[B * P * 4:B * P * 7].view(B, P, 3)
        scl = buf[B * P * 7:].view(B, P, 3)
        if verts.dtype is not torch.float32 or not verts.is_contiguous():
            verts = _f32(verts)
        vt = vert_transforms
        if vt.dtype is not torch.float32 or not vt.is_contiguous():
            vt = _f32(vt)
        rc = _lib.load().gsr_deform_gaussians(
            B, V, self.faces.shape[0], self.N, _ptr(verts), _ptr(vt), _ptr(self.faces),
            _ptr(self.v_rot), 0, _ptr(self.v_scale), 0, _ptr(self.bind), _ptr(self.bary),
            _ptr(self.u_local), 0, _ptr(self.u_rot), 0, _ptr(self.u_scale), 0, _ptr(xyz), _ptr(rot),
            _ptr(scl), _ptr(self.bad), _stream(dev))
        _lib.check(rc, "gsr_deform_gaussians")
        return {"features_color": self.colors.expand(B, -1, -1), "xyz": xyz, "rotation": rot,
                "scaling": scl, "opacity": self.opacity.expand(B, -1, -1),
                "sh_degree": self.sh_degree, "smplx_xyz_deform": verts}

    __call__ = forward

    def bad_index(self):
        return bool(self.bad.item())


def _attr(t, B, n, k, name):
    if tuple(t.shape) == (n, k):
        return _f32(t), 0
    if tuple(t.shape) == (B, n, k):
        return _f32(t), n * k
    raise ValueError(f"{name}: expected [{n},{k}] or [{B},{n},{k}], got {list(t.shape)}")


def deform_inputs(B, verts, vert_transforms, faces, binding_face, face_bary, attrs, bad):
    V, N = verts.shape[1], binding_face.shape[0]
    (vr, s_vr), (vs, s_vs), (ul, s_ul), (ur, s_ur), (us, s_us) = (
        _attr(t, B, n, k, name) for t, n, k, name in zip(
            attrs, (V, V, N, N, N), (4, 3, 3, 4, 3),
            ("vtx_rotations", "vtx_scales", "local_pos", "uv_rotations", "uv_scales")))
    keep = (verts, vert_transforms, faces, binding_face, face_bary, vr, vs, ul, ur, us, bad)
    _dev_check(*keep)
    di = _lib.DeformInputs(V, faces.shape[0], N, 0, _ptr(verts), _ptr(vert_transforms), _ptr(faces), _ptr(vr), s_vr,
                           _ptr(vs), s_vs, _ptr(binding_face), _ptr(face_bary), _ptr(ul), s_ul, _ptr(ur), s_ur,
                           _ptr(us), s_us, _ptr(bad))
    return di, keep


class _DeformGaussians(torch.autograd.Function):

    @staticmethod
    def forward(ctx, verts, vert_transforms, faces, binding_face, face_bary, bad, *attrs):
        B, V = verts.shape[:2]
        N = binding_face.shape[0]
        P = V + N
        di, keep = deform_inputs(B, verts, vert_transforms, faces, binding_face, face_bary, attrs, bad)
        buf = torch.empty((B * P * 10,), dtype=torch.float32, device=verts.device)
        rot = buf[:B * P * 4].view(B, P, 4)
        xyz = buf[B * P * 4:B * P * 7].view(B, P, 3)
        scl = buf[B * P * 7:].view(B, P, 3)
        rc = _lib.load().gsr_deform_gaussians(
            B, V, di.F, N, di.verts, di.vert_transforms, di.faces, di.vtx_rotations, di.vtx_rot_stride,
            di.vtx_scales, di.vtx_scale_stride, di.binding_face, di.face_bary, di.local_xyz, di.local_stride,
            di.uv_rotations, di.uv_rot_stride, di.uv_scales, di.uv_scale_stride, _ptr(xyz), _ptr(rot), _ptr(scl),
            di.bad_index_flag, _stream(verts.device))
        _lib.check(rc, "gsr_deform_gaussians")
        ctx.save_for_backward(*keep[:10])
        ctx.bad = bad
        ctx.attr_shapes = [tuple(a.shape) for a in attrs]
        return xyz, rot, scl

    @staticmethod
    def backward(ctx, g_xyz, g_rot, g_scl):
        verts, vt, faces, bind, bary = ctx.saved_tensors[:5]
        attrs = ctx.saved_tensors[5:]
        B, dev = verts.shape[0], verts.device
        di, keep = deform_inputs(B, verts, vt, faces, bind, bary, attrs, ctx.bad)
        need = ctx.needs_input_grad[6:]
        outs = [torch.zeros(shp, dtype=torch.float32, device=dev) if nd else None
                for shp, nd in zip(ctx.attr_shapes, need)]
        dgr = _lib.DeformGrads(*[None if o is None else o.data_ptr() for o in outs])
        P = verts.shape[1] + bind.shape[0]
        ups = [torch.zeros((B, P, k), dtype=torch.float32, device=dev) if g is None else _f32(g)
               for g, k in zip((g_xyz, g_rot, g_scl), (3, 4, 3))]
        rc = _lib.load().gsr_deform_gaussians_backward(B, ctypes.byref(di), _ptr(ups[0]), _ptr(ups[1]),
                                                       _ptr(ups[2]), ctypes.byref(dgr), _stream(dev))
        _lib.check(rc, "gsr_deform_gaussians_backward")
        del keep
        return (None,) * 6 + tuple(outs)


def deform_gaussians(verts, vert_transforms, faces, binding_face, face_bary, vtx_rotations, vtx_scales,
                     local_pos, uv_rotations, uv_scales, bad_index_flag=None):
    if verts.requires_grad or vert_transforms.requires_grad:
        raise NotImplementedError("deform_gaussians has no gradient for verts / vert_transforms "
                                  "(detach them: the mesh is a constant of the canonical attributes' backward)")
    _dev_check(verts, vert_transforms)
    if verts.dim() != 3 or tuple(vert_transforms.shape) != tuple(verts.shape[:2]) + (4, 4):
        raise ValueError("verts / vert_transforms: expected [B,V,3] / [B,V,4,4]")
    faces = faces.detach().to(torch.int32).contiguous()
    bind = binding_face.detach().reshape(-1).to(torch.int32).contiguous()
    bary = _f32(face_bary.reshape(-1, 3))
    bad = bad_index_flag if bad_index_flag is not None else torch.zeros(1, dtype=torch.int32, device=verts.device)
    return _DeformGaussians.apply(_f32(verts), _f32(vert_transforms), faces, bind, bary, bad, vtx_rotations,
                                  vtx_scales, local_pos, uv_rotations, uv_scales)


def _host(x):
    return x.detach().cpu().numpy() if torch.is_tensor(x) else np.asarray(x)


def tile_base(base_kmajor, stream=None):
    K, M = base_kmajor.shape
    L = _lib.load()
    out = torch.empty((int(L.gsr_lbs_tiled_floats(K, M)),), dtype=torch.float32, device=base_kmajor.device)
    b = base_kmajor.contiguous()
    _lib.check(L.gsr_lbs_tile_bases(K, M, b.data_ptr(), out.data_ptr(), stream or _stream(base_kmajor.device)),
               "gsr_lbs_tile_bases")
    return out


def sparse_lbs_assets(J_regressor, lbs_weights, device):
    jr = np.ascontiguousarray(_host(J_regressor), dtype=np.float32)
    w = np.ascontiguousarray(_host(lbs_weights), dtype=np.float32)
    J, V = jr.shape
    nz = jr != 0
    row = np.concatenate([[0], np.cumsum(nz.sum(1))]).astype(np.int32)
    col = np.nonzero(nz)[1].astype(np.int32)
    val = jr[nz].astype(np.float32)
    t = lambda a: torch.as_tensor(np.ascontiguousarray(a), device=device)
    keep = [t(row), t(col if col.size else np.zeros(1, np.int32)), t(val if val.size else np.zeros(1, np.float32))]
    sp = _lib.LbsSparse(keep[0].data_ptr(), keep[1].data_ptr(), keep[2].data_ptr(), 0, 0, None, None)
    wnz = w != 0
    K = int(wnz.sum(1).max()) if V else 0
    if 1 <= K <= 16:
        order = np.argsort(~wnz, axis=1, kind="stable")[:, :K]
        sj = np.where(np.take_along_axis(wnz, order, 1), order, 0).astype(np.int32)
        sw = np.where(np.take_along_axis(wnz, order, 1), np.take_along_axis(w, sj, 1), 0.0)
        keep += [t(sj.T), t(sw.T.astype(np.float32))]
        sp.skin_k = K
        sp.skin_joint = keep[3].data_ptr()
        sp.skin_weight = keep[4].data_ptr()
    return sp, keep


class EHMDeformer:

    HEAD_REF = (3, 5)
    BODY_REF = (23, 25)

    def __init__(self, body, flame, smplx2flame_ind, l_eyelid, r_eyelid, device="cuda"):
        dev = torch.device(device)
        t = lambda x: torch.as_tensor(np.ascontiguousarray(x), device=dev)
        self.dev = dev
        self.body = {k: (t(v) if k != "parents" else np.asarray(v, np.int32)) for k, v in body.items()}
        self.flame = {k: (t(v) if k != "parents" else np.asarray(v, np.int32)) for k, v in flame.items()}
        for a in (self.body, self.flame):
            a["shapedirs_t"] = _shapedirs_t(a["shapedirs"])
            a["lbs_weights_t"] = _weights_t(a["lbs_weights"])
        self.sparse = {}
        if os.environ.get("GSR_LBS_SPARSE", "1") != "0":
            for name, a in (("body", body), ("flame", flame)):
                self.sparse[name] = sparse_lbs_assets(a["J_regressor"], a["lbs_weights"], dev)
        for name, a in (("body", self.body), ("flame", self.flame)):
            if name in self.sparse:
                sp, keep = self.sparse[name]
                bases = (a["shapedirs_t"], _f32(a["posedirs"]))
                tl = [tile_base(x) if x.numel() else None for x in bases]
                keep += tl
                sp.shapedirs_tiled, sp.posedirs_tiled = (x.data_ptr() if x is not None else None for x in tl)
                (sp.shapedirs_tiled_k, sp.shapedirs_tiled_m), (sp.posedirs_tiled_k, sp.posedirs_tiled_m) = (
                    tuple(x.shape) if x.numel() else (0, 0) for x in bases)
# ... 166 lines not shown
```

guava_renderer_amd/pipeline.py:

```python
import numpy as np
import torch

from .batch import BatchRasterizer
from .deform import EHMDeformer, GaussianDeformer

C = 32


class AvatarPipeline:
    def __init__(self, body, flame, extra, gaussians, B, W, H, R_capacity=None, device="cuda"):
        dev = torch.device(device)
        t = lambda x: torch.as_tensor(np.ascontiguousarray(x), device=dev)
        self.dev = dev
        self.ehm = EHMDeformer(body, flame, extra["smplx2flame_ind"], extra["l_eyelid"],
                               extra["r_eyelid"], device=dev)
        g = gaussians
        V = body["v_template"].shape[0]
        self.gauss = GaussianDeformer(
            {"rotations": t(g["vtx_rotations"]), "scales": t(g["vtx_scales"]),
             "opacities": t(g["opacities"][:V]), "colors": t(g["colors"][:V])},
            {"rotations": t(g["uv_rotations"]), "scales": t(g["uv_scales"]),
             "opacities": t(g["opacities"][V:]), "colors": t(g["colors"][V:]),
             "local_pos": t(g["local_xyz"]), "binding_face": t(g["binding_face"]),
             "face_bary": t(g["face_bary"])}, t(extra["faces"]), apply_rgb_sigmoid=False)
        self.P = self.gauss.V + self.gauss.N
        self.B, self.W, self.H = B, W, H
        self.rast = BatchRasterizer(B, self.P, W, H, R_capacity=R_capacity, device=dev)
        self.bg = torch.zeros((B, C), dtype=torch.float32, device=dev)

    def deform(self, body_params, flame_params):
        e = self.ehm(body_params, flame_params)
        return self.gauss(e["vertices"], e["ver_transform_mat"])

    def render(self, body_params, flame_params, views, projs, tanfov, refine=None, fused=False):
        if fused:
            e = self.ehm(body_params, flame_params)
            col, inv, radii = self.rast.forward_deformed(self.gauss, e["vertices"], e["ver_transform_mat"], views,
                                                         projs, tanfov, self.bg, refine=refine)
            return col, inv, radii, None
        d = self.deform(body_params, flame_params)
        col, inv, radii = self.rast.forward(d["xyz"], self.gauss.colors, self.gauss.opacity,
                                            d["scaling"], d["rotation"], views, projs, tanfov, self.bg,
                                            refine=refine, forward_only=True)
        return col, inv, radii, d
```

include/gsr_deform.h:

```cpp
#ifndef GSR_DEFORM_H
#define GSR_DEFORM_H
#include <stddef.h>
#include <stdint.h>

#include "gsr.h"

#ifdef __cplusplus
extern "C" {
#endif

#define GSR_LBS_MAX_JOINTS 64

size_t gsr_lbs_workspace_bytes(int B, int V, int J, int NB);

int gsr_lbs(int B, int V, int J, int NB, const float* v_template, int64_t v_template_stride,
            const float* betas, const float* shapedirs_t, const float* pose, int pose2rot,
            const float* posedirs, const float* J_regressor, const int32_t* parents_host,
            const float* lbs_weights_t, const float* joints_offset, float* verts,
            float* joints_transformed, float* joints, float* vert_transforms,
            float* joint_transforms, float* v_shaped, char* workspace, void* stream);

typedef struct {
    const int32_t* jreg_row;
    const int32_t* jreg_col;
    const float* jreg_val;
    int32_t skin_k;
    int32_t pad_;
    const int32_t* skin_joint;
    const float* skin_weight;
    const float* shapedirs_tiled;
    const float* posedirs_tiled;
    int32_t shapedirs_tiled_k, shapedirs_tiled_m;
    int32_t posedirs_tiled_k, posedirs_tiled_m;
} GsrLbsSparse;
size_t gsr_lbs_tiled_floats(int K, int M);
int gsr_lbs_tile_bases(int K, int M, const float* base, float* tiled, void* stream);
#define GSR_LBS_SKIN_MAX_K 16

int gsr_lbs_sp(int B, int V, int J, int NB, const float* v_template, int64_t v_template_stride,
               const float* betas, const float* shapedirs_t, const float* pose, int pose2rot,
               const float* posedirs, const float* J_regressor, const int32_t* parents_host,
               const float* lbs_weights_t, const float* joints_offset, float* verts,
               float* joints_transformed, float* joints, float* vert_transforms,
               float* joint_transforms, float* v_shaped, char* workspace, const GsrLbsSparse* sp,
               void* stream);

int gsr_blend_joints(int B, int V, int J, int NB, const float* v_template, int64_t v_template_stride,
                     const float* betas, const float* shapedirs_t, const float* J_regressor,
                     const float* joints_offset, float* v_shaped, float* joints, void* stream);
int gsr_blend_joints_sp(int B, int V, int J, int NB, const float* v_template, int64_t v_template_stride,
                        const float* betas, const float* shapedirs_t, const float* J_regressor,
                        const float* joints_offset, float* v_shaped, float* joints, const GsrLbsSparse* sp,
                        void* stream);

int gsr_splice_head(int B, int V_body, int N_head, const int32_t* head_index, const float* head_verts,
                    const float* r_eyelid, const float* l_eyelid, const float* eyelid_params,
                    const float* head_scale, const float* head_joints, int J_head, int hj0, int hj1,
                    const float* body_joints, int J_body, int bj0, int bj1, float* body_v_shaped,
                    uint32_t* bad_index_flag, void* stream);

typedef struct {
    int V, F, N, pad_;
    const float* verts;
    const float* vert_transforms;
    const int32_t* faces;
    const float* vtx_rotations; int64_t vtx_rot_stride;
    const float* vtx_scales; int64_t vtx_scale_stride;
    const int32_t* binding_face;
    const float* face_bary;
    const float* local_xyz; int64_t local_stride;
    const float* uv_rotations; int64_t uv_rot_stride;
    const float* uv_scales; int64_t uv_scale_stride;
    uint32_t* bad_index_flag;
} GsrDeformInputs;
int gsr_forward_batch_deformed(int B, int width, int height, const GsrDeformInputs* dg, const float* colors,
                               int64_t colors_stride, const float* opacities, int64_t opac_stride,
                               float scale_modifier, const float* viewmatrices, const float* projmatrices,
                               const float* tanfov, const float* backgrounds, int64_t bg_stride,
                               char* workspace, int64_t R_capacity, float* out_color, float* out_invdepth,
                               int* radii, int antialiasing, uint32_t numerics, void* stream);
int gsr_forward_batch_deformed_refine(int B, int width, int height, const GsrDeformInputs* dg, const float* colors,
                                      int64_t colors_stride, const float* opacities, int64_t opac_stride,
                                      float scale_modifier, const float* viewmatrices, const float* projmatrices,
                                      const float* tanfov, const float* backgrounds, int64_t bg_stride,
                                      char* workspace, int64_t R_capacity, float* out_color, float* out_invdepth,
                                      int* radii, int antialiasing, const gsr_refine_epilogue* refine,
                                      uint32_t numerics, void* stream);

typedef struct {
    const float* src;
    float* dst;
    int64_t src_stride;
    int64_t dst_stride;
    int32_t width;
    int32_t pad_;
} GsrRowSegment;
#define GSR_PACK_MAX_SEGMENTS 16

int gsr_pack_rows(int B, int nseg, const GsrRowSegment* segs, void* stream);

typedef struct {
    int32_t V, J, NB, pad_;
    const float* v_template;
    const float* shapedirs_t;
    const float* posedirs;
    const float* J_regressor;
    const float* lbs_weights_t;
    const int32_t* parents_host;
    const GsrLbsSparse* sparse;
} GsrEhmModel;
typedef struct {
    GsrEhmModel flame, body;
    const int32_t* head_index;
    const float* l_eyelid;
    const float* r_eyelid;
    int32_t N_head;
    int32_t hj0, hj1, bj0, bj1;
    int32_t pad_;
    uint32_t* bad_index_flag;
} GsrEhm;
typedef struct {
    const float* p;
    int64_t row_stride;
    int32_t width, pad_;
} GsrEhmParam;
enum {
    GSR_EHM_FLAME_SHAPE = 0, GSR_EHM_FLAME_EXPR, GSR_EHM_FLAME_JAW, GSR_EHM_FLAME_EYES, GSR_EHM_FLAME_EYELID,
    GSR_EHM_BODY_SHAPE, GSR_EHM_BODY_EXP, GSR_EHM_BODY_GLOBAL, GSR_EHM_BODY_POSE, GSR_EHM_BODY_LHAND,
    GSR_EHM_BODY_RHAND, GSR_EHM_BODY_HEAD_SCALE, GSR_EHM_BODY_JOINTS_OFFSET, GSR_EHM_NPARAM
};
typedef struct {
    float* vertices;
    float* joints;
    float* joints_transform;
    float* ver_transform_mat;
    float* joint_transform_mat;
} GsrEhmOutputs;
size_t gsr_ehm_workspace_bytes(const GsrEhm* ehm, int B);
int gsr_ehm_forward(const GsrEhm* ehm, int B, const GsrEhmParam* params, const GsrEhmOutputs* out,
                    char* workspace, void* stream);

int gsr_deform_gaussians(int B, int V, int F, int N, const float* verts,
                         const float* vert_transforms, const int32_t* faces,
                         const float* vtx_rotations, int64_t vtx_rot_stride,
                         const float* vtx_scales, int64_t vtx_scale_stride,
                         const int32_t* binding_face, const float* face_bary,
                         const float* local_xyz, int64_t local_stride,
                         const float* uv_rotations, int64_t uv_rot_stride,
                         const float* uv_scales, int64_t uv_scale_stride, float* means3D,
                         float* rotations, float* scales, uint32_t* bad_index_flag, void* stream);

typedef struct {
    float* vtx_rotations;
    float* vtx_scales;
    float* local_xyz;
    float* uv_rotations;
    float* uv_scales;
} GsrDeformGrads;

int gsr_deform_gaussians_backward(int B, const GsrDeformInputs* dg, const float* dL_dmeans3D,
                                  const float* dL_drotations, const float* dL_dscales,
                                  const GsrDeformGrads* grads, void* stream);

int gsr_backward_batch_deformed(int B, int width, int height, const GsrDeformInputs* dg, const float* means3D,
                                const float* rotations, const float* scales, const float* colors,
                                int64_t colors_stride, const float* opacities, int64_t opac_stride,
                                float scale_modifier, const float* viewmatrices, const float* projmatrices,
                                const float* tanfov, const float* backgrounds, int64_t bg_stride,
                                char* workspace, int64_t R_capacity, const float* dL_dpix,
                                const float* dL_dinvdepth, float* dL_dopacity, float* dL_dcolor,
                                const GsrDeformGrads* grads, int antialiasing, uint32_t numerics,
                                void* stream);

#ifdef __cplusplus
}
#endif
#endif
```

Baseline: 18480 frames/s.

## Fuse Gaussian assembly into projection with cached binding rows

```diff
diff --git a/guava_renderer_amd/_lib.py b/guava_renderer_amd/_lib.py
--- a/guava_renderer_amd/_lib.py
+++ b/guava_renderer_amd/_lib.py
@@ -16,7 +16,7 @@
            "gsr_lbs_workspace_bytes", "gsr_lbs", "gsr_lbs_sp", "gsr_blend_joints", "gsr_blend_joints_sp",
            "gsr_lbs_tiled_floats", "gsr_lbs_tile_bases",
            "gsr_scratch_geometry", "gsr_scratch_binning", "gsr_scratch_image", "gsr_forward_batch_deformed",
-           "gsr_forward_batch_deformed_refine",
+           "gsr_forward_batch_deformed_refine", "gsr_binding_rows", "gsr_forward_batch_assembled",
            "gsr_splice_head",
            "gsr_pack_rows", "gsr_deform_gaussians", "gsr_ehm_workspace_bytes", "gsr_ehm_forward",
            "gsr_deform_gaussians_backward", "gsr_backward_batch_deformed",
@@ -74,6 +74,10 @@
                 ("vtx_scale_stride", _i64), ("binding_face", _vp), ("face_bary", _vp), ("local_xyz", _vp),
                 ("local_stride", _i64), ("uv_rotations", _vp), ("uv_rot_stride", _i64), ("uv_scales", _vp),
                 ("uv_scale_stride", _i64), ("bad_index_flag", _vp)]
+
+
+class BindingRows(ctypes.Structure):
+    _fields_ = [("V", _i), ("F", _i), ("N", _i), ("pad_", _i), ("rows", _vp)]
 
 
 class DeformGrads(ctypes.Structure):
@@ -191,6 +195,12 @@
     L.gsr_forward_batch_deformed_refine.argtypes = list(L.gsr_forward_batch_deformed.argtypes[:-2]) + [
         ctypes.POINTER(RefineEpilogue), _u32, _vp]
     L.gsr_forward_batch_deformed_refine.restype = _i
+    L.gsr_binding_rows.argtypes = [_i, _i, _i, _vp, _vp, _vp, _vp, _vp]
+    L.gsr_binding_rows.restype = _i
+    L.gsr_forward_batch_assembled.argtypes = [_i, _i, _i, ctypes.POINTER(DeformInputs), ctypes.POINTER(BindingRows),
+                                              _vp, _vp, _vp] + list(
+        L.gsr_forward_batch_deformed.argtypes[4:-2]) + [ctypes.POINTER(RefineEpilogue), _u32, _vp]
+    L.gsr_forward_batch_assembled.restype = _i
     L.gsr_render_variant.argtypes = [_i, _u32, _i]
     L.gsr_render_variant.restype = _i
     L.gsr_refine_prepare.argtypes = [_i, _vp, _vp, _i, _i, _vp, _vp]
diff --git a/guava_renderer_amd/batch.py b/guava_renderer_amd/batch.py
--- a/guava_renderer_amd/batch.py
+++ b/guava_renderer_amd/batch.py
@@ -159,7 +159,7 @@
         return self.out_color, self.out_invdepth, self.radii
 
     def forward_deformed(self, deformer, verts, vert_transforms, viewmatrices, projmatrices, tanfov, backgrounds,
-                         scale_modifier=1.0, antialiasing=False, numerics=None, refine=None):
+                         scale_modifier=1.0, antialiasing=False, numerics=None, refine=None, assets_out=None):
         self.poll()
         nm = self.numerics if numerics is None else int(numerics)
         self._fwd_only = True
@@ -181,20 +181,25 @@
                                dfm.faces.data_ptr(), dfm.v_rot.data_ptr(), 0, dfm.v_scale.data_ptr(), 0,
                                dfm.bind.data_ptr(), dfm.bary.data_ptr(), dfm.u_local.data_ptr(), 0,
                                dfm.u_rot.data_ptr(), 0, dfm.u_scale.data_ptr(), 0, dfm.bad.data_ptr())
-        args = (B, self.W, self.H, ctypes.byref(di), head[6], head[7], head[8], head[9], float(scale_modifier),
-                v, pm, tf, bg, bs, self.workspace.data_ptr(), self.R_capacity, self.out_color.data_ptr(),
-                self.out_invdepth.data_ptr(), self.radii.data_ptr(), int(bool(antialiasing)))
-        if refine is None:
-            _lib.check(self.L.gsr_forward_batch_deformed(*args, nm, self._stream()), "gsr_forward_batch_deformed")
-        else:
+        outs = (None, None, None)
+        if assets_out is not None:
+            for t_, k, name in zip(assets_out, (3, 4, 3), ("xyz", "rotation", "scaling")):
+                if (tuple(t_.shape) != (B, P, k) or t_.dtype != torch.float32 or t_.device != self.device
+                        or not t_.is_contiguous()):
+                    raise ValueError(f"assets_out {name}: expected a contiguous float32 [{B},{P},{k}] on {self.device}")
+            outs = tuple(t_.data_ptr() for t_ in assets_out)
+        colors_ptr, bg_ptr, ep = head[6], bg, None
+        if refine is not None:
             pc = refine.prepare(keep[1], self._stream())
             pb = refine.prepare(keep[8].reshape(-1, C), self._stream(), cache=False)
-            args = list(args)
-            args[4] = pc.data_ptr()
-            args[12] = pb.data_ptr()
-            ep = refine.epilogue(B, self.H, self.W)
-            _lib.check(self.L.gsr_forward_batch_deformed_refine(*args, ctypes.byref(ep), nm, self._stream()),
-                       "gsr_forward_batch_deformed_refine")
+            colors_ptr, bg_ptr = pc.data_ptr(), pb.data_ptr()
+            ep = ctypes.byref(refine.epilogue(B, self.H, self.W))
+        rc = self.L.gsr_forward_batch_assembled(
+            B, self.W, self.H, ctypes.byref(di), ctypes.byref(dfm.binding_rows()), *outs, colors_ptr, head[7],
+            head[8], head[9], float(scale_modifier), v, pm, tf, bg_ptr, bs, self.workspace.data_ptr(),
+            self.R_capacity, self.out_color.data_ptr(), self.out_invdepth.data_ptr(), self.radii.data_ptr(),
+            int(bool(antialiasing)), ep, nm, self._stream())
+        _lib.check(rc, "gsr_forward_batch_assembled, as gsr_forward_batch_deformed" + ("" if refine is None else "_refine"))
         del keep, vb, vt
         self._after_forward()
         return self.out_color, self.out_invdepth, self.radii
diff --git a/guava_renderer_amd/csrc/capi.hip b/guava_renderer_amd/csrc/capi.hip
--- a/guava_renderer_amd/csrc/capi.hip
+++ b/guava_renderer_amd/csrc/capi.hip
@@ -192,8 +192,9 @@
     return align_up(off) + 256;
 }
 
-void launch_deform_preprocess(const Dims& d, const Inputs& in, const GeomArena& g, const Outputs& o,
-                              const GsrDeformInputs& dg, hipStream_t s);
+void launch_assemble_project(const Dims& d, const Inputs& in, const GeomArena& g, const Outputs& o,
+                             const GsrDeformInputs& dg, const void* rows, float* means, float* rots,
+                             float* scales, hipStream_t s);
 void launch_preprocess_bwd_deformed(const Dims& d, const Inputs& in, const GeomArena& g, const Grads& gr,
                                     const GsrDeformInputs& dg, const GsrDeformGrads& dgr, hipStream_t s);
 int check_deform_inputs(int B, const GsrDeformInputs* dg, const char* who);
@@ -560,7 +561,9 @@
                               const float* tanfov, const float* backgrounds, int64_t bg_stride,
                               char* workspace, int64_t R_capacity, float* out_color, float* out_invdepth,
                               int* radii, int antialiasing, const gsr_refine_epilogue* refine,
-                              uint32_t numerics, const GsrDeformInputs* dg, hipStream_t s) {
+                              uint32_t numerics, const GsrDeformInputs* dg, hipStream_t s,
+                              const void* binding_rows = nullptr, float* assets_means = nullptr,
+                              float* assets_rot = nullptr, float* assets_scales = nullptr) {
     if (numerics & ~kForwardBatchKnown) return fail(GSR_ERR_ARG, "unknown numerics flags");
     if (refine) {
         if (!refine->out_refine || refine->n_out < 1 || refine->keep_channels < 0 ||
@@ -608,7 +611,7 @@
     if (!in.zero_ctrl) HIP_TRY(hipMemsetAsync(g.ctrl, 0, ctrl_words(d) * 4, s));
     if (dg) {
         StageTimer st_(0, s);
-        launch_deform_preprocess(d, in, g, o, *dg, s);
+        launch_assemble_project(d, in, g, o, *dg, binding_rows, assets_means, assets_rot, assets_scales, s);
     } else {
         StageTimer st_(0, s);
         launch_preprocess(d, in, g, o, s);
@@ -659,13 +662,7 @@
                                              antialiasing, nullptr, numerics, stream);
 }
 
-int gsr_forward_batch_deformed_refine(int B, int width, int height, const GsrDeformInputs* dg, const float* colors,
-                                      int64_t colors_stride, const float* opacities, int64_t opac_stride,
-                                      float scale_modifier, const float* viewmatrices, const float* projmatrices,
-                                      const float* tanfov, const float* backgrounds, int64_t bg_stride,
-                                      char* workspace, int64_t R_capacity, float* out_color, float* out_invdepth,
-                                      int* radii, int antialiasing, const gsr_refine_epilogue* refine,
-                                      uint32_t numerics, void* stream) {
+static int check_avatar_forward(const GsrDeformInputs* dg) {
     if (!dg || dg->V < 0 || dg->N < 0 || dg->F < 0 || dg->V + dg->N == 0 || !dg->verts)
         return fail(GSR_ERR_ARG, "gsr_forward_batch_deformed: bad deform inputs");
     if (dg->V > 0 && (!dg->vert_transforms || !dg->vtx_rotations || !dg->vtx_scales))
@@ -678,10 +675,45 @@
         bad_stride(dg->local_stride, 3LL * dg->N) || bad_stride(dg->uv_rot_stride, 4LL * dg->N) ||
         bad_stride(dg->uv_scale_stride, 3LL * dg->N))
         return fail(GSR_ERR_ARG, "gsr_forward_batch_deformed: strides must be 0 or a whole frame");
+    return 0;
+}
+
+int gsr_forward_batch_deformed_refine(int B, int width, int height, const GsrDeformInputs* dg, const float* colors,
+                                      int64_t colors_stride, const float* opacities, int64_t opac_stride,
+                                      float scale_modifier, const float* viewmatrices, const float* projmatrices,
+                                      const float* tanfov, const float* backgrounds, int64_t bg_stride,
+                                      char* workspace, int64_t R_capacity, float* out_color, float* out_invdepth,
+                                      int* radii, int antialiasing, const gsr_refine_epilogue* refine,
+                                      uint32_t numerics, void* stream) {
+    if (const int rc = check_avatar_forward(dg)) return rc;
     return forward_batch_impl(B, dg->V + dg->N, width, height, nullptr, 0, colors, colors_stride, opacities,
                               opac_stride, nullptr, 0, nullptr, 0, scale_modifier, viewmatrices, projmatrices,
                               tanfov, backgrounds, bg_stride, workspace, R_capacity, out_color, out_invdepth, radii,
                               antialiasing, refine, numerics | GSR_FORWARD_ONLY, dg, (hipStream_t)stream);
+}
+
+int gsr_forward_batch_assembled(int B, int width, int height, const GsrDeformInputs* dg,
+                                const GsrBindingRows* rows, float* means3D, float* rotations, float* scales,
+                                const float* colors, int64_t colors_stride, const float* opacities,
+                                int64_t opac_stride, float scale_modifier, const float* viewmatrices,
+                                const float* projmatrices, const float* tanfov, const float* backgrounds,
+                                int64_t bg_stride, char* workspace, int64_t R_capacity, float* out_color,
+                                float* out_invdepth, int* radii, int antialiasing,
+                                const gsr_refine_epilogue* refine, uint32_t numerics, void* stream) {
+    if (const int rc = check_avatar_forward(dg)) return rc;
+    if (!rows || rows->V != dg->V || rows->F != dg->F || rows->N != dg->N || (dg->N > 0 && !rows->rows) ||
+        ((uintptr_t)rows->rows & 15) != 0)
+        return fail(GSR_ERR_ARG, "gsr_forward_batch_assembled: binding rows missing or built for another V, F, N");
+    const int nout = (means3D != nullptr) + (rotations != nullptr) + (scales != nullptr);
+    if (nout != 0 && nout != 3)
+        return fail(GSR_ERR_ARG, "gsr_forward_batch_assembled: means3D, rotations, scales are all set or all NULL");
+    if (((uintptr_t)rotations & 15) != 0)
+        return fail(GSR_ERR_ARG, "gsr_forward_batch_assembled: rotations must be 16-byte aligned");
+    return forward_batch_impl(B, dg->V + dg->N, width, height, nullptr, 0, colors, colors_stride, opacities,
+                              opac_stride, nullptr, 0, nullptr, 0, scale_modifier, viewmatrices, projmatrices,
+                              tanfov, backgrounds, bg_stride, workspace, R_capacity, out_color, out_invdepth, radii,
+                              antialiasing, refine, numerics | GSR_FORWARD_ONLY, dg, (hipStream_t)stream,
+                              dg->N > 0 ? rows->rows : nullptr, means3D, rotations, scales);
 }
 
 int gsr_refine_prepare(int n, const float* rows, const float* weight, int n_out, int keep_channels,
diff --git a/guava_renderer_amd/csrc/deform.hip b/guava_renderer_amd/csrc/deform.hip
--- a/guava_renderer_amd/csrc/deform.hip
+++ b/guava_renderer_amd/csrc/deform.hip
@@ -1032,77 +1032,66 @@
     }
 }
 
-__global__ __launch_bounds__(256) void k_deform_preprocess(int fpw, GsrDeformInputs dg, Dims d, Inputs in,
-                                                           GeomArena g, Outputs o) {
-    __shared__ float fr_lds[256 * kFrStride];
-    __shared__ int range[2];
-    const int V = dg.V, F = dg.F, N = dg.N, P = V + N;
-    const int32_t* __restrict__ faces = dg.faces;
-    const int i = blockIdx.x * blockDim.x + threadIdx.x;
-    const bool uv = i >= V && i < P;
-    const int n = i - V;
-    int f = -1, j0 = 0, j1 = 0, j2 = 0;
-    if (uv) {
-        const int bf = dg.binding_face[n];
-        if (bf >= 0 && bf < F) {
-            const int a = faces[3 * bf], c = faces[3 * bf + 1], e = faces[3 * bf + 2];
-            if (a >= 0 && a < V && c >= 0 && c < V && e >= 0 && e < V) { f = bf; j0 = a; j1 = c; j2 = e; }
-        }
-        if (f < 0 && dg.bad_index_flag) atomicOr(dg.bad_index_flag, 1u);
-    }
-    float w0 = 0.f, w1 = 0.f, w2 = 0.f;
-    if (uv) { w0 = dg.face_bary[3 * n]; w1 = dg.face_bary[3 * n + 1]; w2 = dg.face_bary[3 * n + 2]; }
-    if (threadIdx.x == 0) { range[0] = INT_MAX; range[1] = -1; }
-    __syncthreads();
-    if (f >= 0) { atomicMin(&range[0], f); atomicMax(&range[1], f); }
-    __syncthreads();
-    const int fmin = range[0], nf = range[1] - range[0] + 1;
-    const bool shared_frames = range[1] >= 0 && nf <= 256;
-    int t0 = -1, t1 = 0, t2 = 0;
-    if (shared_frames && (int)threadIdx.x < nf) {
-        const int ff = fmin + threadIdx.x;
-        const int a = faces[3 * ff], c = faces[3 * ff + 1], e = faces[3 * ff + 2];
-        if (a >= 0 && a < V && c >= 0 && c < V && e >= 0 && e < V) { t0 = a; t1 = c; t2 = e; }
-    }
-    const int b1 = min(d.B, (int)(blockIdx.y + 1) * fpw);
-    for (int b = blockIdx.y * fpw; b < b1; b++) {
+__global__ __launch_bounds__(256) void k_binding_rows(int V, int F, int N, const int32_t* __restrict__ faces,
+                                                      const int32_t* __restrict__ bind,
+                                                      const float* __restrict__ bary, int4* __restrict__ rows) {
+    const int n = blockIdx.x * blockDim.x + threadIdx.x;
+    if (n >= N) return;
+    const DeformBinding bd = resolve_binding(bind, faces, n, V, F);
+    rows[2 * (int64_t)n] = make_int4(bd.j0, bd.j1, bd.j2, bd.f >= 0 ? 1 : 0);
+    reinterpret_cast<float4*>(rows)[2 * (int64_t)n + 1] = make_float4(bary[3 * n], bary[3 * n + 1], bary[3 * n + 2], 0.f);
+}
+
+__global__ __launch_bounds__(256) void k_assemble_project(GsrDeformInputs dg, const int4* __restrict__ rows,
+                                                          float* __restrict__ means, float* __restrict__ rots,
+                                                          float* __restrict__ scales, Dims d, Inputs in,
+                                                          GeomArena g, Outputs o) {
+    const int V = dg.V, P = V + dg.N;
+    const int b = blockIdx.y;
+    const int i = blockIdx.x * kScanBlock + threadIdx.x;
+    const int64_t gid = (int64_t)b * P + i;
+    for (int k = i; k <= d.NB; k += d.nblk * kScanBlock) g.bcount[(int64_t)b * (d.NB + 1) + k] = 0u;
+    uint32_t tiles = 0;
+    float depth = 0.f;
+    if (i < P) {
         const float* vb = dg.verts + (int64_t)b * V * 3;
-        if (shared_frames) {
-            if (b > (int)blockIdx.y * fpw) __syncthreads();
-            if (t0 >= 0) face_frame(vb, t0, t1, t2, fr_lds + threadIdx.x * kFrStride);
-            __syncthreads();
-        }
-        for (int k = i; k <= d.NB; k += d.nblk * kScanBlock) g.bcount[(int64_t)b * (d.NB + 1) + k] = 0u;
-        const int64_t gid = (int64_t)b * P + i;
-        uint32_t tiles = 0;
-        if (i < P) {
-            float mo[3], so[3], qq[4];
-            if (i < V) {
-                const float4* tv = reinterpret_cast<const float4*>(dg.vert_transforms + ((int64_t)b * V + i) * 16);
-                const float4 r0 = tv[0], r1 = tv[1], r2 = tv[2];
-                const float m[9] = {r0.x, r0.y, r0.z, r1.x, r1.y, r1.z, r2.x, r2.y, r2.z};
-                const float4 qd = rotmat_to_unitquat(m);
-                const float* qv = dg.vtx_rotations + b * dg.vtx_rot_stride + 4 * (int64_t)i;
-                const float4 q = quat_product(qd, make_float4(qv[1], qv[2], qv[3], qv[0]));
-                const float nn = fmaxf(sqrtf(((q.w * q.w + q.x * q.x) + q.y * q.y) + q.z * q.z), 1e-12f);
-                qq[0] = q.w / nn; qq[1] = q.x / nn; qq[2] = q.y / nn; qq[3] = q.z / nn;
-                for (int c = 0; c < 3; c++) {
-                    mo[c] = vb[3 * i + c];
-                    so[c] = dg.vtx_scales[b * dg.vtx_scale_stride + 3 * (int64_t)i + c];
-                }
-            } else if (f < 0) {
+        float mo[3], so[3], qq[4];
+        if (i < V) {
+            const float4* tv = reinterpret_cast<const float4*>(dg.vert_transforms + ((int64_t)b * V + i) * 16);
+            const float4 r0 = tv[0], r1 = tv[1], r2 = tv[2];
+            const float m[9] = {r0.x, r0.y, r0.z, r1.x, r1.y, r1.z, r2.x, r2.y, r2.z};
+            const float4 qd = rotmat_to_unitquat(m);
+            const float* qv = dg.vtx_rotations + b * dg.vtx_rot_stride + 4 * (int64_t)i;
+            const float4 q = quat_product(qd, make_float4(qv[1], qv[2], qv[3], qv[0]));
+            const float nn = fmaxf(sqrtf(((q.w * q.w + q.x * q.x) + q.y * q.y) + q.z * q.z), 1e-12f);
+            qq[0] = q.w / nn; qq[1] = q.x / nn; qq[2] = q.y / nn; qq[3] = q.z / nn;
+            for (int c = 0; c < 3; c++) {
+                mo[c] = vb[3 * i + c];
+                so[c] = dg.vtx_scales[b * dg.vtx_scale_stride + 3 * (int64_t)i + c];
+            }
+        } else {
+            const int n = i - V;
+            int j0, j1, j2;
+            float w0, w1, w2;
+            bool valid;
+            if (rows) {
+                const int4 r = rows[2 * (int64_t)n];
+                const float4 w = reinterpret_cast<const float4*>(rows)[2 * (int64_t)n + 1];
+                j0 = r.x; j1 = r.y; j2 = r.z; valid = r.w != 0;
+                w0 = w.x; w1 = w.y; w2 = w.z;
+            } else {
+                const DeformBinding bd = resolve_binding(dg.binding_face, dg.faces, n, V, dg.F);
+                j0 = bd.j0; j1 = bd.j1; j2 = bd.j2; valid = bd.f >= 0;
+                w0 = dg.face_bary[3 * n]; w1 = dg.face_bary[3 * n + 1]; w2 = dg.face_bary[3 * n + 2];
+            }
+            if (!valid) {
+                if (dg.bad_index_flag && b == 0) atomicOr(dg.bad_index_flag, 1u);
                 const float nan = __int_as_float(0x7fc00000);
                 for (int c = 0; c < 3; c++) { mo[c] = nan; so[c] = nan; }
                 for (int c = 0; c < 4; c++) qq[c] = nan;
             } else {
                 float fr[14];
-                if (shared_frames) {
-                    const float* src = fr_lds + (f - fmin) * kFrStride;
-#pragma unroll
-                    for (int k = 0; k < 14; k++) fr[k] = src[k];
-                } else {
-                    face_frame(vb, j0, j1, j2, fr);
-                }
+                face_frame(vb, j0, j1, j2, fr);
                 const float s = fr[9];
                 const float* qu = dg.uv_rotations + b * dg.uv_rot_stride + 4 * (int64_t)n;
                 const float4 q = quat_product(make_float4(fr[10], fr[11], fr[12], fr[13]),
@@ -1119,22 +1108,23 @@
                 const float* us = dg.uv_scales + b * dg.uv_scale_stride + 3 * (int64_t)n;
                 for (int c = 0; c < 3; c++) so[c] = us[c] * s;
             }
-            tiles = preprocess_one(d, in, g, o, b, gid, mo, nullptr, so, qq, in.opac[in.s_opac * b + i]);
-        }
-        preprocess_block_sums(d, g, b, blockIdx.x, tiles, gid);
+        }
+        if (means) {
+            reinterpret_cast<float4*>(rots)[gid] = make_float4(qq[0], qq[1], qq[2], qq[3]);
+            for (int c = 0; c < 3; c++) { means[3 * gid + c] = mo[c]; scales[3 * gid + c] = so[c]; }
+        }
+        tiles = preprocess_one(d, in, g, o, b, gid, mo, nullptr, so, qq, in.opac[in.s_opac * b + i], &depth);
     }
     zero_ctrl_words(d, in, g);
-}
-
-void launch_deform_preprocess(const Dims& d, const Inputs& in, const GeomArena& g, const Outputs& o,
-                              const GsrDeformInputs& dg, hipStream_t s) {
+    preprocess_block_sums(d, g, b, blockIdx.x, tiles, depth);
+}
+
+void launch_assemble_project(const Dims& d, const Inputs& in, const GeomArena& g, const Outputs& o,
+                             const GsrDeformInputs& dg, const void* rows, float* means, float* rots,
+                             float* scales, hipStream_t s) {
     if (d.P == 0 || d.B == 0) return;
-    static const int fpw = [] {
-        const int v = tune_env("GSR_FUSED_FRAMES", 4);
-        return v >= 1 && v <= 64 ? v : 1;
-    }();
-    hipLaunchKernelGGL(k_deform_preprocess, dim3(d.nblk, (d.B + fpw - 1) / fpw), dim3(256), 0, s, fpw, dg, d, in,
-                       g, o);
+    hipLaunchKernelGGL(k_assemble_project, dim3(d.nblk, d.B), dim3(kScanBlock), 0, s, dg,
+                       reinterpret_cast<const int4*>(rows), means, rots, scales, d, in, g, o);
 }
 
 __global__ __launch_bounds__(256) void k_deform_gaussians_bwd(int B, int fpw, GsrDeformInputs dg,
@@ -1829,6 +1819,18 @@
     return hip_check("deform_gaussians");
 }
 
+int gsr_binding_rows(int V, int F, int N, const int32_t* faces, const int32_t* binding_face,
+                     const float* face_bary, void* rows, void* stream) {
+    if (V < 0 || F < 0 || N < 0) return api_fail(GSR_ERR_ARG, "gsr_binding_rows: bad sizes");
+    if (N == 0) return 0;
+    if (!faces || !binding_face || !face_bary || !rows || F == 0)
+        return api_fail(GSR_ERR_ARG, "gsr_binding_rows: null pointer or no faces");
+    if (((uintptr_t)rows & 15) != 0) return api_fail(GSR_ERR_ARG, "gsr_binding_rows: rows must be 16-byte aligned");
+    hipLaunchKernelGGL(k_binding_rows, dim3((N + 255) / 256), dim3(256), 0, (hipStream_t)stream, V, F, N, faces,
+                       binding_face, face_bary, reinterpret_cast<int4*>(rows));
+    return hip_check("binding_rows");
+}
+
 int gsr_deform_gaussians_backward(int B, const GsrDeformInputs* dg, const float* dL_dmeans3D,
                                   const float* dL_drotations, const float* dL_dscales,
                                   const GsrDeformGrads* grads, void* stream) {
diff --git a/guava_renderer_amd/csrc/preprocess.hip b/guava_renderer_amd/csrc/preprocess.hip
--- a/guava_renderer_amd/csrc/preprocess.hip
+++ b/guava_renderer_amd/csrc/preprocess.hip
@@ -8,6 +8,7 @@
     const int64_t gid = (int64_t)b * d.P + i;
     for (int k = i; k <= d.NB; k += d.nblk * kScanBlock) g.bcount[(int64_t)b * (d.NB + 1) + k] = 0u;
     uint32_t tiles = 0;
+    float depth = 0.f;
     if (i < d.P) {
         const float* pm = in.means3D + in.s_means * b + 3 * (int64_t)i;
         const float p[3] = {pm[0], pm[1], pm[2]};
@@ -19,10 +20,10 @@
             sc[0] = sp[0]; sc[1] = sp[1]; sc[2] = sp[2];
             q[0] = rp[0]; q[1] = rp[1]; q[2] = rp[2]; q[3] = rp[3];
         }
-        tiles = preprocess_one(d, in, g, o, b, gid, p, cp, sc, q, in.opac[in.s_opac * b + i]);
+        tiles = preprocess_one(d, in, g, o, b, gid, p, cp, sc, q, in.opac[in.s_opac * b + i], &depth);
     }
     zero_ctrl_words(d, in, g);
-    preprocess_block_sums(d, g, b, blockIdx.x, tiles, gid);
+    preprocess_block_sums(d, g, b, blockIdx.x, tiles, depth);
 }
 
 void launch_preprocess(const Dims& d, const Inputs& in, const GeomArena& g, const Outputs& o,
diff --git a/guava_renderer_amd/csrc/preprocess_dev.h b/guava_renderer_amd/csrc/preprocess_dev.h
--- a/guava_renderer_amd/csrc/preprocess_dev.h
+++ b/guava_renderer_amd/csrc/preprocess_dev.h
@@ -21,7 +21,7 @@
 __device__ __forceinline__ uint32_t preprocess_one(const Dims& d, const Inputs& in, const GeomArena& g,
                                                    const Outputs& o, int b, int64_t gid, const float p[3],
                                                    const float* cp, const float sc[3], const float q[4],
-                                                   float op) {
+                                                   float op, float* depth) {
     uint32_t tiles = 0;
     const float* view = in.view + 16 * b;
     const float* proj = in.proj + 16 * b;
@@ -88,6 +88,7 @@
             const uint32_t nt = (rmax[0] - rmin[0]) * (rmax[1] - rmin[1]);
             if (nt != 0) {
                 g.depth[gid] = pv[2];
+                *depth = pv[2];
                 if (!in.fwd_only) {
                     g.invdepth[gid] = 1.0f / pv[2];
                     g.means2D[gid] = make_float2(pix0, pix1);
@@ -110,10 +111,10 @@
 }
 
 __device__ __forceinline__ void preprocess_block_sums(const Dims& d, const GeomArena& g, int b, int blk_x,
-                                                      uint32_t tiles, int64_t gid) {
+                                                      uint32_t tiles, float depth) {
     __shared__ uint32_t red[3][kScanBlock / 64];
     uint32_t v = tiles;
-    const uint32_t key = tiles ? __float_as_uint(g.depth[gid]) : 0u;
+    const uint32_t key = tiles ? __float_as_uint(depth) : 0u;
     uint32_t kmax = key, nkmax = tiles ? ~key : 0u;
 #pragma unroll
     for (int off = 32; off > 0; off >>= 1) {
@@ -140,7 +141,6 @@
         g.blockkey[2 * blk] = km;
         g.blockkey[2 * blk + 1] = nkm;
     }
-    __syncthreads();
 }
 
 
diff --git a/guava_renderer_amd/deform.py b/guava_renderer_amd/deform.py
--- a/guava_renderer_amd/deform.py
+++ b/guava_renderer_amd/deform.py
@@ -178,18 +178,40 @@
         self.opacity = torch.cat([sq(va["opacities"]), sq(ua["opacities"])], 0).contiguous()
         self.sh_degree = sh_degree
         self.bad = torch.zeros(1, dtype=torch.int32, device=self.faces.device)
+        self._rows = None
+        self.binding_rows()
+
+    def binding_rows(self):
+        key = tuple((t.data_ptr(), t._version) for t in (self.faces, self.bind, self.bary))
+        if self._rows is None or self._rows[0] != key:
+            dev = self.faces.device
+            rows = torch.empty((max(self.N, 1), 8), dtype=torch.int32, device=dev)
+            F = self.faces.shape[0]
+            if self.N:
+                _lib.check(_lib.load().gsr_binding_rows(self.V, F, self.N, _ptr(self.faces), _ptr(self.bind),
+                                                        _ptr(self.bary), _ptr(rows), _stream(dev)),
+                           "gsr_binding_rows")
+            self._rows = (key, rows, _lib.BindingRows(self.V, F, self.N, 0, rows.data_ptr()))
+        return self._rows[2]
+
+    def assets_buffer(self, B, device):
+        P = self.V + self.N
+        buf = torch.empty((B * P * 10,), dtype=torch.float32, device=device)
+        return (buf[:B * P * 4].view(B, P, 4), buf[B * P * 4:B * P * 7].view(B, P, 3),
+                buf[B * P * 7:].view(B, P, 3))
+
+    def assets_dict(self, B, xyz, rot, scl, verts):
+        return {"features_color": self.colors.expand(B, -1, -1), "xyz": xyz, "rotation": rot,
+                "scaling": scl, "opacity": self.opacity.expand(B, -1, -1),
+                "sh_degree": self.sh_degree, "smplx_xyz_deform": verts}
 
     def forward(self, verts, vert_transforms):
         _dev_check(verts, vert_transforms)
         B, V = verts.shape[:2]
         if V != self.V:
             raise RuntimeError(f"expected {self.V} vertices, got {V}")
-        P = self.V + self.N
         dev = verts.device
-        buf = torch.empty((B * P * 10,), dtype=torch.float32, device=dev)
-        rot = buf[:B * P * 4].view(B, P, 4)
-        xyz = buf[B * P * 4:B * P * 7].view(B, P, 3)
-        scl = buf[B * P * 7:].view(B, P, 3)
+        rot, xyz, scl = self.assets_buffer(B, dev)
         if verts.dtype is not torch.float32 or not verts.is_contiguous():
             verts = _f32(verts)
         vt = vert_transforms
@@ -201,9 +223,7 @@
             _ptr(self.u_local), 0, _ptr(self.u_rot), 0, _ptr(self.u_scale), 0, _ptr(xyz), _ptr(rot),
             _ptr(scl), _ptr(self.bad), _stream(dev))
         _lib.check(rc, "gsr_deform_gaussians")
-        return {"features_color": self.colors.expand(B, -1, -1), "xyz": xyz, "rotation": rot,
-                "scaling": scl, "opacity": self.opacity.expand(B, -1, -1),
-                "sh_degree": self.sh_degree, "smplx_xyz_deform": verts}
+        return self.assets_dict(B, xyz, rot, scl, verts)
 
     __call__ = forward
 
diff --git a/guava_renderer_amd/pipeline.py b/guava_renderer_amd/pipeline.py
--- a/guava_renderer_amd/pipeline.py
+++ b/guava_renderer_amd/pipeline.py
@@ -33,13 +33,13 @@
         return self.gauss(e["vertices"], e["ver_transform_mat"])
 
     def render(self, body_params, flame_params, views, projs, tanfov, refine=None, fused=False):
-        if fused:
-            e = self.ehm(body_params, flame_params)
-            col, inv, radii = self.rast.forward_deformed(self.gauss, e["vertices"], e["ver_transform_mat"], views,
-                                                         projs, tanfov, self.bg, refine=refine)
-            return col, inv, radii, None
-        d = self.deform(body_params, flame_params)
-        col, inv, radii = self.rast.forward(d["xyz"], self.gauss.colors, self.gauss.opacity,
-                                            d["scaling"], d["rotation"], views, projs, tanfov, self.bg,
-                                            refine=refine, forward_only=True)
+        e = self.ehm(body_params, flame_params)
+        verts, T = e["vertices"], e["ver_transform_mat"]
+        d = outs = None
+        if not fused:
+            rot, xyz, scl = self.gauss.assets_buffer(self.B, self.dev)
+            outs = (xyz, rot, scl)
+            d = self.gauss.assets_dict(self.B, xyz, rot, scl, verts)
+        col, inv, radii = self.rast.forward_deformed(self.gauss, verts, T, views, projs, tanfov, self.bg,
+                                                     refine=refine, assets_out=outs)
         return col, inv, radii, d
diff --git a/include/gsr_deform.h b/include/gsr_deform.h
--- a/include/gsr_deform.h
+++ b/include/gsr_deform.h
@@ -88,6 +88,22 @@
                                       uint32_t numerics, void* stream);
 
 typedef struct {
+    int V, F, N, pad_;
+    const void* rows;
+} GsrBindingRows;
+int gsr_binding_rows(int V, int F, int N, const int32_t* faces, const int32_t* binding_face,
+                     const float* face_bary, void* rows, void* stream);
+
+int gsr_forward_batch_assembled(int B, int width, int height, const GsrDeformInputs* dg,
+                                const GsrBindingRows* rows, float* means3D, float* rotations, float* scales,
+                                const float* colors, int64_t colors_stride, const float* opacities,
+                                int64_t opac_stride, float scale_modifier, const float* viewmatrices,
+                                const float* projmatrices, const float* tanfov, const float* backgrounds,
+                                int64_t bg_stride, char* workspace, int64_t R_capacity, float* out_color,
+                                float* out_invdepth, int* radii, int antialiasing,
+                                const gsr_refine_epilogue* refine, uint32_t numerics, void* stream);
+
+typedef struct {
     const float* src;
     float* dst;
     int64_t src_stride;
```

New measurement: 18610 frames/s, median of 6. No clear change (+0.7%).
